# HTDerekLiu/surface_multigrid_code

Hardware: AMD Instinct MI355X
Metric: V-cycles/sec + fine-level SpMV GB/s (% HBM peak), 1M-vert mesh fp64 (higher is better)
Workload: dtype f64; 1 GPU; C3: bunny_15K_init x3 midpoint subdivision, 1011330 verts, 5 levels, M_bary+0.01(-L), fp64; n_verts=1011330, nnz=7079298, levels=5, smoother=gs, rhs_columns_per_gpu=1, parallelism=single GPU

## Files before the change

include/smg.h:

```cpp
#ifndef SMG_H
#define SMG_H

#ifdef __cplusplus
extern "C" {
#endif

#define SMG_VERSION 508

enum {
    SMG_OK = 0,
    SMG_ERR_INVALID = -1,
    SMG_ERR_NO_DEVICE = -2,
    SMG_ERR_HIP = -3,
    SMG_ERR_NONFINITE = -4,
    SMG_ERR_ALLOC = -5,
    SMG_ERR_IO = -6,
    SMG_ERR_REDUCE = -7
};

enum { SMG_HOST = 0, SMG_DEVICE = 1 };

enum { SMG_DEC_QSLIM = 0, SMG_DEC_MIDPOINT = 1, SMG_DEC_VERTEX_REMOVAL = 2 };

enum { SMG_SMOOTH_GS = 0, SMG_SMOOTH_JACOBI = 1, SMG_SMOOTH_HYBRID = 2, SMG_SMOOTH_CHEBYSHEV = 3, SMG_SMOOTH_HYBRID_CHEBYSHEV = 4 };

typedef struct smg_hierarchy smg_hierarchy;

typedef struct {
    double tol;
    int max_iter;
    int pre, post;
    int verbosity;
    int check_every;
    int use_graph;
    int precision;
    int smoother;
    double omega;
    int jacobi_max_rows;
    double cheby_fraction;
} smg_solve_opts;
void smg_solve_opts_default(smg_solve_opts *o);

int smg_version(void);
const char *smg_last_error(void);
int smg_device_count(void);
long long smg_device_bytes_live(void);
int smg_debug_device_bytes(const smg_hierarchy *h, char *buf, int cap);

smg_hierarchy *smg_hierarchy_create(int n_levels);
void smg_hierarchy_destroy(smg_hierarchy *h);
int smg_hierarchy_levels(const smg_hierarchy *h);
int smg_hierarchy_set_stream(smg_hierarchy *h, void *hip_stream);
int smg_hierarchy_set_smoother(smg_hierarchy *h, int smoother, double omega, int jacobi_max_rows);
int smg_hierarchy_set_chebyshev(smg_hierarchy *h, double cheby_fraction);
double smg_level_spectral_bound(const smg_hierarchy *h, int lv);
int smg_level_set_prolong(smg_hierarchy *h, int lv, int n_fine, int n_coarse, const int *rowptr, const int *col,
                          const double *val);
int smg_level_set_prolong_csc(smg_hierarchy *h, int lv, int n_fine, int n_coarse, const int *colptr,
                              const int *rowidx, const double *val);
int smg_level_set_mesh(smg_hierarchy *h, int lv, const double *V, int nV, const int *F, int nF);
int smg_level_get_mesh(const smg_hierarchy *h, int lv, int *nV, int *nF, double *V, int *F);

int smg_mg_precompute(const double *V, int nV, const int *F, int nF, float ratio, int nVCoarsest, int dec_type,
                      smg_hierarchy **out);
int smg_mg_precompute_capped(const double *V, int nV, const int *F, int nF, float ratio, int nVCoarsest, int dec_type,
                             float absorption_cap, smg_hierarchy **out);
int smg_mg_precompute_logged(const double *V, int nV, const int *F, int nF, float ratio, int nVCoarsest, int dec_type,
                             float absorption_cap, int keep_log, smg_hierarchy **out);
int smg_query_coarse_to_fine(const smg_hierarchy *h, int lv, int n, const int *face, const double *bary, int *out_face,
                             double *out_bary);
int smg_query_fine_to_coarse(const smg_hierarchy *h, int lv, int n, const int *face, const double *bary, int *out_face,
                             double *out_bary);
int smg_mg_precompute_subdiv(const double *V, int nV, const int *F, int nF, int n_sub, float ratio, int nVCoarsest,
                             int n_extra_levels, smg_hierarchy **out, double *V_out, int *F_out);

int smg_mg_precompute_block(const double *V, int nV, const int *F, int nF, float ratio, int nVCoarsest, int dec_type,
                            smg_hierarchy **out);
int smg_hierarchy_set_block_mode(smg_hierarchy *h, int mode);
int smg_hierarchy_block_size(const smg_hierarchy *h);
int smg_level_block_stats(const smg_hierarchy *h, int lv, long *n_blocks, long *n_block_slots, int *n_vertex_colors);
int smg_level_get_block_image(const smg_hierarchy *h, int lv, int *n_slices, int *n_panel_cols, int *slice_row, int *slice_off, int *slice_w,
                              int *col, double *val);
int smg_hierarchy_set_block_gs(smg_hierarchy *h, int min_rows);
int smg_level_get_block_gs_order(smg_hierarchy *h, int lv, int k, int *n_blocks, int *n_colors, int *color_ptr, int *blk_ptr, int *rows, double *stats);
int smg_hierarchy_set_wave_gs(smg_hierarchy *h, int mode);
int smg_hierarchy_set_memory_lean(smg_hierarchy *h, int on);
int smg_level_get_wave_gs_order(smg_hierarchy *h, int lv, int k, int *n_pieces, int *n_colors, int *color_ptr, int *piece_ptr, int *rows, double *stats);
int smg_hierarchy_create_union(const smg_hierarchy *const *members, int m, smg_hierarchy **out);
int smg_union_members(const smg_hierarchy *h);
int smg_union_member_rows(const smg_hierarchy *h, int member, int *first, int *count);
// ... 52 lines not shown
} smg_membrane_params;
void smg_membrane_params_default(smg_membrane_params *p);
typedef struct smg_membrane smg_membrane;
int smg_membrane_create(const smg_hierarchy *h, const double *V, int nV, const int *F, int nF, const smg_membrane_params *p, smg_membrane **out);
void smg_membrane_destroy(smg_membrane *m);
long long smg_membrane_device_bytes(const smg_membrane *m);
int smg_membrane_set_state(smg_membrane *m, const double *pos, const double *qdot, int memspace);
int smg_membrane_get_state(smg_membrane *m, double *pos, double *qdot, int memspace);
int smg_membrane_set_solver(smg_membrane *m, int pcg);
int smg_membrane_step(smg_membrane *m, const smg_solve_opts *opts, double *objective_his, double *alpha, int *cycles, int *n_newton);
int smg_membrane_lists(const int *F, int nF, int nV, int *n_blocks, int *n_contrib, int *bptr, int *bcol, int *c_ptr, int *c_src);
int smg_membrane_faces_host(const double *V0, const double *P, int nV, const int *F, int nF, const smg_membrane_params *p, int fix, double *W,
                            double *G, double *H);

int smg_solve_begin(smg_hierarchy *h, const double *RHS, int ld_rhs, const double *known_val, int ld_kv,
                    const double *z0, int ld_z0, int k, int memspace, const smg_solve_opts *opts);
int smg_solve_iter_residual(smg_hierarchy *h, double *d_sumsq);
int smg_solve_iter_cycle(smg_hierarchy *h, const double *d_sumsq);
int smg_solve_iter_cycle_speculative(smg_hierarchy *h);
int smg_solve_iter_commit(smg_hierarchy *h, const double *d_sumsq);
int smg_solve_poll(smg_hierarchy *h, int *done, int *n_his);
int smg_solve_end(smg_hierarchy *h, double *z, int ld_z, int memspace, double *r_his, int *n_his, int *converged);

typedef int (*smg_reduce_fn)(double *d_sumsq, int count, void *hip_stream, void *ctx);
int smg_solve_sharded(smg_hierarchy *h, const double *RHS, int ld_rhs, const double *known_val, int ld_kv, const double *z0,
                      int ld_z0, int k_local, int memspace, const smg_solve_opts *opts, smg_reduce_fn reduce, void *ctx,
                      double *z, int ld_z, double *r_his, int *n_his, int *converged);

int smg_level_rows(const smg_hierarchy *h, int lv);
int smg_vcycle(smg_hierarchy *h, const double *B, int pre, int post, int lv, double *u, int k);
int smg_apply_A(smg_hierarchy *h, int lv, const double *u, int k, double *Au);
int smg_restrict(smg_hierarchy *h, int lv, const double *x, int k, double *Rx);
int smg_prolong(smg_hierarchy *h, int lv, const double *x, int k, double *Px);
int smg_relax(smg_hierarchy *h, int lv, const double *B, int k, int iters, double *u);
int smg_coarse_solve(smg_hierarchy *h, const double *B, int k, double *u);
int smg_residual_norm(smg_hierarchy *h, int lv, const double *B, const double *u, int k, double *norm);

int smg_raw_spmv(smg_hierarchy *h, int lv, int mode, const double *x, const double *b, double *y, int k);
int smg_raw_relax(smg_hierarchy *h, int lv, const double *b, double *u, int k, int iters);
int smg_raw_spmv_f32(smg_hierarchy *h, int lv, const float *x, float *y, int k);
int smg_raw_outer_iteration(smg_hierarchy *h, int n_iter);
int smg_synchronize(smg_hierarchy *h);
int smg_bench_vcycle(smg_hierarchy *h, int lv, int k, int pre, int post, int reps, double *us_per_cycle);
int smg_bench_relax(smg_hierarchy *h, int lv, int k, int sweeps, int reps, double *us_per_call);

int smg_level_get_matrix(const smg_hierarchy *h, int lv, int which, int internal, int *n_rows, int *n_cols, int *nnz,
                         int *rowptr, int *col, double *val);
int smg_level_get_perm(const smg_hierarchy *h, int lv, int *perm);
int smg_level_get_colors(const smg_hierarchy *h, int lv, int *n_colors, int *color_ptr );
int smg_level_get_Adiag(const smg_hierarchy *h, int lv, double *diag);
int smg_get_unknown(const smg_hierarchy *h, int *n_unknown, int *unknown );
int smg_level_sell_stats(const smg_hierarchy *h, int lv, int which, long *stored, long *padded, int *n_slices);
int smg_level_first_colour_rows(const smg_hierarchy *h, int lv);
long smg_level_spmv_bytes(const smg_hierarchy *h, int lv, int k);
long smg_vcycle_bytes(const smg_hierarchy *h, int k, int pre, int post);

int smg_debug_check_tiling_plan(smg_hierarchy *h, int lv, int sweeps, int tile_rows, int *n_tiles, int *max_ext_rows, double *redundancy,
                                double *max_abs_diff);
int smg_debug_check_block_gs_plan(smg_hierarchy *h, int lv, int block_rows, int *n_blocks, int *n_colors, double *rim, double *fill, double *max_abs_diff);
int smg_debug_check_wave_gs_plan(smg_hierarchy *h, int lv, int piece_rows, int pieces_mode, int *n_pieces, int *n_colors, double *stats, double *max_abs_diff);
int smg_debug_raise_coarse_stall(smg_hierarchy *h);
int smg_debug_schur_solve_host(int n, const int *ptr, const int *col, const double *val, const double *b, double *x, int *n_blocks, int *n_sep);
int smg_debug_schur_partition(const smg_hierarchy *h, int *n_blocks, int *n_sep, int *block_of_row);
int smg_debug_check_sparse_cholesky(int n, const int *rowptr, const int *col, const double *val, long *factor_entries, int *dependency_depth,
                                    double *rel_residual);

int smg_debug_dense_geneig_host(int n, const double *A, const double *B, double *evals, double *V);

int smg_debug_eig_gram(int n, int m, int nb_a, const double *Sa, int nb_b, const double *Sb, const double *w, int sym, int done, double *G,
                       int *groups, int *guard_bad);
int smg_debug_eig_combine(int n, int m, int nb, const double *S, const double *AS, const double *C, int make_p, int done, double *X, double *AX,
                          double *P, double *AP, int *guard_bad);
int smg_debug_eig_residual(int n, int m, const double *X, const double *AX, const double *mass, const double *lam, int f32, int done, double *b0,
                           double *u0, float *b32, float *u32, double *res, int *groups, int *guard_bad);
enum { SMG_KRY_DOTS_ZR_ZQ = 0, SMG_KRY_DIRECTION = 1, SMG_KRY_DOTS_PQ = 2, SMG_KRY_STEP_DECIDE = 3, SMG_KRY_PRECOND_IN = 4, SMG_KRY_WIDEN = 5 };
int smg_debug_krylov(int op, int n, int k, double *v0, double *v1, double *v2, double *v3, float *e, double *s, int *restart, double tol, int done,
                     double *ctrl_d, int *ctrl_i, int *groups, int *guard_bad);
enum { SMG_F32_A = 0, SMG_F32_RESID = 1, SMG_F32_RESTRICT = 2, SMG_F32_PROLONG_ADD = 3, SMG_F32_RELAX = 4, SMG_F32_COARSE = 5, SMG_F32_VCYCLE = 6 };
int smg_debug_cycle_f32(smg_hierarchy *h, int op, int lv, int k, int pre, int post, int done, const float *in0, const float *in1, float *out,
                        int *inputs_changed);
enum { SMG_F32_RESIDUAL_TO_F32 = 0, SMG_F32_ADD_CORRECTION = 1 };
int smg_debug_convert_f32(smg_hierarchy *h, int op, int k, int done, const double *in64, const float *in32, double *out64, float *out_b32,
                          float *out_u32, int *inputs_changed);
enum { SMG_GEO_BASIS = 0, SMG_GEO_SCATTER = 1, SMG_GEO_DIVERGENCE = 2, SMG_GEO_SHIFT = 3 };
int smg_debug_geodesics(int op, int n, int nF, int k, const int *F, const int *m_ptr, const int *m_idx, const int *src_ptr, const int *src,
                        const double *in, double *W, double *Af, double *out, int ld_out, int *guard_bad);
enum { SMG_ARAP_COVARIANCE = 0, SMG_ARAP_ROTATIONS = 1, SMG_ARAP_RHS = 2, SMG_ARAP_VERTEX_ENERGY = 3, SMG_ARAP_ENERGY = 4 };
int smg_debug_arap(int op, int n, const int *rowptr, const int *col, const double *w, const double *P0, const double *P, const double *R_in,
                   double *out, int *guard_hits);

enum { SMG_MEM_REST = 0, SMG_MEM_FACES_RAW = 1, SMG_MEM_FACES = 2, SMG_MEM_ENERGY = 3, SMG_MEM_PRESSURE = 4, SMG_MEM_MATRIX = 5,
       SMG_MEM_GRADIENT = 6, SMG_MEM_OBJECTIVE = 7 };
int smg_debug_membrane(int op, int nV, int nF, const int *F, const double *V0, const double *P, const double *in, const smg_membrane_params *p,
                       double *out, int *guard_hits);

int smg_prof_enable(smg_hierarchy *h, int on);
int smg_prof_reset(smg_hierarchy *h);
int smg_prof_count(smg_hierarchy *h);
int smg_prof_get(smg_hierarchy *h, int idx, char *name, int name_cap, long *count, double *total_ms);

int smg_mesh_read(const char *path, double **V, int *nV, int **F, int *nF);
void smg_free(void *p);
int smg_mesh_normalize_unit_area(double *V, int nV, const int *F, int nF);
int smg_mesh_cotmatrix(const double *V, int nV, const int *F, int nF, int *nnz, int *rowptr, int *col, double *val);
int smg_mesh_massmatrix(const double *V, int nV, const int *F, int nF, int voronoi, double *diag);
int smg_mesh_boundary_loop(const int *F, int nF, int nV, int *loop, int *n_loop);
int smg_mesh_midpoint_upsample(int nV, const int *F, int nF, int *nE, int *S_rowptr, int *S_col, double *S_val,
                               int *NF);
int smg_mesh_torus(int nu, int nv, double R, double r, double *V, int *F);

#ifdef __cplusplus
}
#endif
#endif
```

surface_multigrid_code_amd/_lib.py:

```python
import ctypes as C
import os

HERE = os.path.dirname(os.path.abspath(__file__))
LIB_PATH = os.environ.get("SMG_LIB") or os.path.join(HERE, "lib", "libsmg.so")

SMG_HOST, SMG_DEVICE = 0, 1


class SolveOptsC(C.Structure):
    _fields_ = [("tol", C.c_double), ("max_iter", C.c_int), ("pre", C.c_int), ("post", C.c_int),
                ("verbosity", C.c_int), ("check_every", C.c_int), ("use_graph", C.c_int), ("precision", C.c_int),
                ("smoother", C.c_int), ("omega", C.c_double), ("jacobi_max_rows", C.c_int), ("cheby_fraction", C.c_double)]


class MembraneParamsC(C.Structure):
    _fields_ = [("young", C.c_double), ("poisson", C.c_double), ("thickness", C.c_double), ("mass_scale", C.c_double), ("dt", C.c_double),
                ("pressure", C.c_double), ("newton_iters", C.c_int), ("ls_c", C.c_double), ("ls_shrink", C.c_double),
                ("ls_min_alpha", C.c_double), ("eig_floor", C.c_double), ("eig_value", C.c_double)]


_lib = None


REDUCE_FN = C.CFUNCTYPE(C.c_int, C.c_void_p, C.c_int, C.c_void_p, C.c_void_p)


def load():
    global _lib
    if _lib is not None:
        return _lib
    if not os.path.exists(LIB_PATH):
        raise ImportError("libsmg.so not built: run `python -m surface_multigrid_code_amd.build` "
                          "(expected at %s); there is no CPU fallback" % LIB_PATH)
    L = C.CDLL(LIB_PATH, mode=C.RTLD_GLOBAL)
    ip, dp, vp, lp, fp = C.POINTER(C.c_int), C.POINTER(C.c_double), C.c_void_p, C.POINTER(C.c_long), C.POINTER(C.c_float)
    i, d, f = C.c_int, C.c_double, C.c_float
    sig = {
        "smg_version": (i, []),
        "smg_last_error": (C.c_char_p, []),
        "smg_device_count": (i, []),
        "smg_device_bytes_live": (C.c_longlong, []),
        "smg_solve_opts_default": (None, [C.POINTER(SolveOptsC)]),
        "smg_hierarchy_create": (vp, [i]),
        "smg_hierarchy_destroy": (None, [vp]),
        "smg_hierarchy_levels": (i, [vp]),
        "smg_hierarchy_set_stream": (i, [vp, vp]),
        "smg_hierarchy_set_smoother": (i, [vp, i, d, i]),
        "smg_hierarchy_set_chebyshev": (i, [vp, d]),
        "smg_level_spectral_bound": (d, [vp, i]),
        "smg_level_set_prolong": (i, [vp, i, i, i, ip, ip, dp]),
        "smg_level_set_prolong_csc": (i, [vp, i, i, i, ip, ip, dp]),
        "smg_level_set_mesh": (i, [vp, i, dp, i, ip, i]),
        "smg_level_get_mesh": (i, [vp, i, ip, ip, dp, ip]),
        "smg_mg_precompute": (i, [dp, i, ip, i, f, i, i, C.POINTER(vp)]),
        "smg_mg_precompute_capped": (i, [dp, i, ip, i, f, i, i, f, C.POINTER(vp)]),
        "smg_mg_precompute_logged": (i, [dp, i, ip, i, f, i, i, f, i, C.POINTER(vp)]),
        "smg_query_coarse_to_fine": (i, [vp, i, i, ip, dp, ip, dp]),
        "smg_query_fine_to_coarse": (i, [vp, i, i, ip, dp, ip, dp]),
        "smg_mg_precompute_block": (i, [dp, i, ip, i, f, i, i, C.POINTER(vp)]),
        "smg_hierarchy_save": (i, [vp, C.c_char_p]),
        "smg_hierarchy_load": (i, [C.c_char_p, C.POINTER(vp)]),
        "smg_mg_precompute_subdiv": (i, [dp, i, ip, i, i, f, i, i, C.POINTER(vp), dp, ip]),
        "smg_precompute": (i, [vp, i, ip, ip, dp, ip, i]),
        "smg_precompute_values_device": (i, [vp, vp]),
        "smg_assembler_create": (i, [ip, i, i, C.POINTER(vp)]),
        "smg_assembler_destroy": (None, [vp]),
        "smg_assembler_pattern": (i, [vp, ip, ip, ip]),
        "smg_assemble": (i, [vp, vp, i, d, d, vp, vp, vp, vp]),
        "smg_solve": (i, [vp, vp, i, vp, i, vp, i, i, i, C.POINTER(SolveOptsC), vp, i, dp, ip, ip]),
        "smg_solve_pcg": (i, [vp, vp, i, vp, i, vp, i, i, i, C.POINTER(SolveOptsC), vp, i, dp, ip, ip]),
        "smg_eigs": (i, [vp, vp, i, i, vp, i, i, C.POINTER(SolveOptsC), C.c_ulonglong, dp, vp, i, dp, ip, ip]),
        "smg_debug_dense_geneig_host": (i, [i, dp, dp, dp, dp]),
        "smg_debug_eig_gram": (i, [i, i, i, dp, i, dp, dp, i, i, dp, ip, ip]),
        "smg_debug_eig_combine": (i, [i, i, i, dp, dp, dp, i, i, dp, dp, dp, dp, ip]),
        "smg_debug_eig_residual": (i, [i, i, dp, dp, dp, dp, i, i, dp, dp, fp, fp, dp, ip, ip]),
        "smg_debug_krylov": (i, [i, i, i, dp, dp, dp, dp, fp, dp, ip, d, i, dp, ip, ip, ip]),
        "smg_debug_cycle_f32": (i, [vp, i, i, i, i, i, i, fp, fp, fp, ip]),
        "smg_debug_convert_f32": (i, [vp, i, i, i, dp, fp, dp, fp, fp, ip]),
        "smg_debug_geodesics": (i, [i, i, i, i, ip, ip, ip, ip, ip, dp, dp, dp, dp, i, ip]),
        "smg_geodesics_create": (i, [vp, dp, i, ip, i, d, i, C.POINTER(vp)]),
        "smg_geodesics_destroy": (None, [vp]),
        "smg_geodesics_time": (d, [vp]),
        "smg_geodesics_set_solver": (i, [vp, i, i]),
        "smg_geodesics_device_bytes": (C.c_longlong, [vp]),
        "smg_geodesics_solve": (i, [vp, i, ip, ip, i, C.POINTER(SolveOptsC), C.POINTER(SolveOptsC), vp, i, ip]),
        "smg_debug_arap": (i, [i, i, ip, ip, dp, dp, dp, dp, dp, ip]),
        "smg_arap_create": (i, [vp, dp, i, ip, i, ip, i, C.POINTER(vp)]),
        "smg_arap_destroy": (None, [vp]),
        "smg_arap_set_solver": (i, [vp, i]),
        "smg_arap_device_bytes": (C.c_longlong, [vp]),
        "smg_arap_solve": (i, [vp, vp, i, vp, i, i, i, d, C.POINTER(SolveOptsC), vp, i, dp, ip, ip]),
        "smg_debug_membrane": (i, [i, i, i, ip, dp, dp, dp, C.POINTER(MembraneParamsC), dp, ip]),
        "smg_membrane_params_default": (None, [C.POINTER(MembraneParamsC)]),
        "smg_membrane_create": (i, [vp, dp, i, ip, i, C.POINTER(MembraneParamsC), C.POINTER(vp)]),
        "smg_membrane_destroy": (None, [vp]),
        "smg_membrane_device_bytes": (C.c_longlong, [vp]),
        "smg_membrane_set_state": (i, [vp, vp, vp, i]),
        "smg_membrane_get_state": (i, [vp, vp, vp, i]),
        "smg_membrane_set_solver": (i, [vp, i]),
        "smg_membrane_step": (i, [vp, C.POINTER(SolveOptsC), dp, dp, ip, ip]),
        "smg_membrane_lists": (i, [ip, i, i, ip, ip, ip, ip, ip, ip]),
        "smg_membrane_faces_host": (i, [dp, dp, i, ip, i, C.POINTER(MembraneParamsC), i, dp, dp, dp]),
        "smg_solve_sharded": (i, [vp, vp, i, vp, i, vp, i, i, i, C.POINTER(SolveOptsC), REDUCE_FN, vp, vp, i, dp, ip, ip]),
        "smg_solve_begin": (i, [vp, vp, i, vp, i, vp, i, i, i, C.POINTER(SolveOptsC)]),
        "smg_solve_iter_residual": (i, [vp, vp]),
        "smg_solve_iter_cycle": (i, [vp, vp]),
        "smg_solve_iter_cycle_speculative": (i, [vp]),
        "smg_solve_iter_commit": (i, [vp, vp]),
        "smg_solve_poll": (i, [vp, ip, ip]),
        "smg_solve_end": (i, [vp, vp, i, i, dp, ip, ip]),
        "smg_level_rows": (i, [vp, i]),
        "smg_vcycle": (i, [vp, dp, i, i, i, dp, i]),
        "smg_apply_A": (i, [vp, i, dp, i, dp]),
        "smg_restrict": (i, [vp, i, dp, i, dp]),
        "smg_prolong": (i, [vp, i, dp, i, dp]),
        "smg_relax": (i, [vp, i, dp, i, i, dp]),
        "smg_coarse_solve": (i, [vp, dp, i, dp]),
        "smg_residual_norm": (i, [vp, i, dp, dp, i, dp]),
        "smg_raw_spmv": (i, [vp, i, i, vp, vp, vp, i]),
        "smg_raw_relax": (i, [vp, i, vp, vp, i, i]),
        "smg_raw_spmv_f32": (i, [vp, i, vp, vp, i]),
        "smg_raw_outer_iteration": (i, [vp, i]),
        "smg_synchronize": (i, [vp]),
        "smg_bench_vcycle": (i, [vp, i, i, i, i, i, dp]),
        "smg_bench_relax": (i, [vp, i, i, i, i, dp]),
        "smg_level_get_matrix": (i, [vp, i, i, i, ip, ip, ip, ip, ip, dp]),
        "smg_level_get_perm": (i, [vp, i, ip]),
        "smg_level_get_colors": (i, [vp, i, ip, ip]),
        "smg_level_get_Adiag": (i, [vp, i, dp]),
        "smg_get_unknown": (i, [vp, ip, ip]),
        "smg_level_sell_stats": (i, [vp, i, i, lp, lp, ip]),
        "smg_level_first_colour_rows": (i, [vp, i]),
        "smg_debug_check_tiling_plan": (i, [vp, i, i, i, ip, ip, dp, dp]),
        "smg_debug_check_sparse_cholesky": (i, [i, ip, ip, dp, lp, ip, dp]),
        "smg_hierarchy_set_coarse_dense_max": (i, [vp, i]),
        "smg_hierarchy_set_coarse_schur": (i, [vp, i, i]),
        "smg_debug_schur_solve_host": (i, [i, ip, ip, dp, dp, dp, ip, ip]),
        "smg_debug_schur_partition": (i, [vp, ip, ip, ip]),
        "smg_hierarchy_set_block_gs": (i, [vp, i]),
        "smg_hierarchy_set_wave_gs": (i, [vp, i]),
        "smg_hierarchy_set_memory_lean": (i, [vp, i]),
        "smg_hierarchy_create_union": (i, [C.POINTER(vp), i, C.POINTER(vp)]),
        "smg_union_members": (i, [vp]),
        "smg_union_member_rows": (i, [vp, i, ip, ip]),
        "smg_union_get_history": (i, [vp, i, dp, i, ip, ip]),
        "smg_debug_device_bytes": (i, [vp, C.c_char_p, i]),
        "smg_level_get_wave_gs_order": (i, [vp, i, i, ip, ip, ip, ip, ip, dp]),
        "smg_debug_check_wave_gs_plan": (i, [vp, i, i, i, ip, ip, dp, dp]),
        "smg_debug_raise_coarse_stall": (i, [vp]),
        "smg_debug_check_block_gs_plan": (i, [vp, i, i, ip, ip, dp, dp, dp]),
        "smg_level_get_block_gs_order": (i, [vp, i, i, ip, ip, ip, ip, ip, dp]),
        "smg_hierarchy_coarse_solver": (i, [vp, lp]),
        "smg_hierarchy_set_block_mode": (i, [vp, i]),
        "smg_hierarchy_block_size": (i, [vp]),
        "smg_level_block_stats": (i, [vp, i, lp, lp, ip]),
        "smg_level_get_block_image": (i, [vp, i, ip, ip, ip, ip, ip, ip, dp]),
        "smg_level_spmv_bytes": (C.c_long, [vp, i, i]),
        "smg_vcycle_bytes": (C.c_long, [vp, i, i, i]),
        "smg_prof_enable": (i, [vp, i]),
        "smg_prof_reset": (i, [vp]),
        "smg_prof_count": (i, [vp]),
# ... 22 lines not shown
```

surface_multigrid_code_amd/csrc/smg_cycle.cpp:

```cpp
#include <hip/hip_runtime.h>

#include <algorithm>
#include <chrono>
#include <cmath>
#include <cstdarg>
#include <cstdio>
#include <cstdlib>
#include <cstring>
#include <functional>
#include <memory>
#include <numeric>
#include <string>
#include <thread>
#include <vector>

#include "smg_internal.hpp"

using namespace smg;


int smg::ensure_work(smg_hierarchy* h, int k)
{
    const int L = h->n_levels;
    if (k > h->kcap) {
// ... 172 lines not shown
            const double rho_new = 1.0 / (2.0 * sigma - rho);
            out[s].c1 = rho_new * rho;
            out[s].c2 = 2.0 * rho_new / delta;
            rho = rho_new;
        }
    }
}

template <typename T> struct Prec;
static inline int coarse_cols(const smg_hierarchy* h, int k) { return (h->coarse_cols > 0 && h->coarse_cols < k) ? h->coarse_cols : k; }

template <> struct Prec<double> {
    static double* b(Level& L) { return L.b.p; }
    static double* u(Level& L) { return L.u.p; }
    static double* r(Level& L) { return L.r.p; }
    static double* t(Level& L) { return L.t.p; }
    static double* d(Level& L) { return L.d.p; }
    static void set_d(FirstColour& fc, Level& L) { fc.d = L.d.p; }
    static const SellDev& A(Level& L) { return L.dA.view; }
    static const SellDev& G(Level& L) { return L.gs_on_transpose ? L.dAT.view : L.dA.view; }
    static const SellDev& P(Level& L) { return L.dP.view; }
    static const SellDev& PT(Level& L) { return L.dPT.view; }
    static bool has_vals(const SellDev& V) { return V.val != nullptr; }
    static hipError_t sell(SellMode m, const SellDev& V, int s0, int s1, const double* x, const double* bb, double* y, int k, const Ctrl* ctrl,
                           hipStream_t st, double* zero_rows = nullptr, const FirstColour* first = nullptr, double omega = 1.0)
    { return launch_sell(m, V, s0, s1, x, bb, y, k, ctrl, nullptr, nullptr, st, zero_rows, first, omega); }
    static hipError_t coarse(smg_hierarchy* h, Level& L, int k, const Ctrl* ctrl)
    {
        if (h->union_m > 0) return launch_blockdiag_gemv_add(h->un.view, h->d_Ainv.p, h->nc, L.b.p, L.u.p, k, ctrl, h->stream);
        if (h->coarse_sparse) return launch_sparse_coarse_solve(h->c_view, L.b.p, L.u.p, k, ctrl, h->stream);
        if (h->coarse_schur) return launch_schur_solve(h->sch.view, L.b.p, L.u.p, k, ctrl, h->stream);
        return launch_dense_gemv_add(h->d_Ainv.p, h->nc, h->nc_pad, L.b.p, L.u.p, coarse_cols(h, k), k, ctrl, h->stream, h->d_sympart.p);
    }
    static hipError_t opA(smg_hierarchy* h, Level& L, bool smoother_image, SellMode m, int s0, int s1, const double* x, const double* bb, double* y, int k,
                          const Ctrl* ctrl, const FirstColour* fc = nullptr, double omega = 1.0)
    {
        if (h->bs == 3) {
            const Bsr3Dev& V = (smoother_image && L.gs_on_transpose) ? L.bAT.view : L.bA.view;
            return launch_bsr3(m, V, s0, s1 < 0 ? V.n_slices : s1, x, bb, y, k, ctrl, nullptr, nullptr, h->stream, omega, fc ? fc->c1 : 0.0, fc ? fc->d : nullptr);
        }
        const SellDev& V = smoother_image ? G(L) : A(L);
        return sell(m, V, s0, s1 < 0 ? V.n_slices : s1, x, bb, y, k, ctrl, h->stream, nullptr, fc, omega);
    }
};
template <> struct Prec<float> {
    static float* b(Level& L) { return L.b32.p; }
    static float* u(Level& L) { return L.u32.p; }
    static float* r(Level& L) { return L.r32.p; }
    static float* t(Level& L) { return L.t32.p; }
    static float* d(Level& L) { return L.d32.p; }
    static void set_d(FirstColour& fc, Level& L) { fc.df = L.d32.p; }
    static const SellDev& A(Level& L) { return L.dA32; }
    static const SellDev& G(Level& L) { return L.gs_on_transpose ? L.dAT32 : L.dA32; }
    static const SellDev& P(Level& L) { return L.dP32; }
    static const SellDev& PT(Level& L) { return L.dPT32; }
    static bool has_vals(const SellDev& V) { return V.valf != nullptr; }
    static hipError_t sell(SellMode m, const SellDev& V, int s0, int s1, const float* x, const float* bb, float* y, int k, const Ctrl* ctrl,
                           hipStream_t st, float* zero_rows = nullptr, const FirstColour* first = nullptr, double omega = 1.0)
    { return launch_sell_f32(m, V, s0, s1, x, bb, y, k, ctrl, st, zero_rows, first, omega); }
    static hipError_t coarse(smg_hierarchy* h, Level& L, int k, const Ctrl* ctrl)
    {
        if (h->coarse_schur) return launch_schur_solve_f32(h->sch.view, L.b32.p, L.u32.p, k, ctrl, h->stream);
        return launch_dense_gemv_add_f32(h->d_Ainv32.p, h->nc, h->nc_pad, L.b32.p, L.u32.p, coarse_cols(h, k), k, ctrl, h->stream, (float*)h->d_sympart.p);
    }
    static hipError_t opA(smg_hierarchy* h, Level& L, bool smoother_image, SellMode m, int s0, int s1, const float* x, const float* bb, float* y, int k,
                          const Ctrl* ctrl, const FirstColour* fc = nullptr, double omega = 1.0)
    {
        if (h->bs == 3) {
            const Bsr3Dev& V = (smoother_image && L.gs_on_transpose) ? L.bAT.view : L.bA.view;
            return launch_bsr3_f32(m, V, s0, s1 < 0 ? V.n_slices : s1, x, bb, y, k, ctrl, h->stream, omega, fc ? fc->c1 : 0.0, fc ? fc->df : nullptr);
        }
        const SellDev& V = smoother_image ? G(L) : A(L);
        return sell(m, V, s0, s1 < 0 ? V.n_slices : s1, x, bb, y, k, ctrl, h->stream, nullptr, fc, omega);
    }
};

static const std::vector<int>& colour_slices(const smg_hierarchy* h, const Level& Lv)
{
    if (h->bs == 3) return (Lv.gs_on_transpose ? Lv.bAT : Lv.bA).color_slice_ptr;
    return (Lv.gs_on_transpose ? Lv.dAT : Lv.dA).color_slice_ptr;
}

template <typename T>
static int enqueue_gs(smg_hierarchy* h, int lv, const SweepPlan& sp, const T* b, T* u, int k, int iters, const Ctrl* ctrl, int first = FIRST_NONE, T* t = nullptr)
{
    Level& Lv = h->lv[lv];
    ProfGuard pg(h, "MG: relaxation");
    if (const WgsBuf* W = sp.wave) {
        for (int it = 0; it < iters; it++)
            for (size_t c = 0; c + 1 < W->color_ptr.size(); c++)
                HIPCHK(launch_wgs(W->view, W->color_ptr[c], W->color_ptr[c + 1], (const double*)b, (double*)u, k, ctrl, h->stream));
        return SMG_OK;
    }
    if (const BgsBuf* Q = sp.block) {
        for (int it = 0; it < iters; it++)
            for (size_t c = 0; c + 1 < Q->color_ptr.size(); c++)
                HIPCHK(launch_bgs(Q->view, Q->color_ptr[c], Q->color_ptr[c + 1], (const double*)b, (double*)u, k, ctrl, h->stream));
        return SMG_OK;
    }
    const std::vector<int>& cs = colour_slices(h, Lv);
    for (int it = first == FIRST_SWEEP ? 1 : 0; it < iters; it++)
        for (size_t c = (it == 0 && first == FIRST_LAUNCH) ? 1 : 0; c + 1 < cs.size(); c++) {
            if (it == 1 && first == FIRST_SWEEP) HIPCHK(Prec<T>::sell(SELL_GS_OOP, Prec<T>::G(Lv), cs[c], cs[c + 1], t, b, u, k, ctrl, h->stream));
            else HIPCHK(Prec<T>::opA(h, Lv, true, SELL_GS, cs[c], cs[c + 1], u, b, u, k, ctrl));
        }
    return SMG_OK;
}

template <typename T>
static int enqueue_gs_tiled(smg_hierarchy* h, const TiledDev& plan, const T* b, T* const buf[2], int* cur, int k, const Ctrl* ctrl)
{
    ProfGuard pg(h, "MG: relaxation");
    HIPCHK(launch_tiled_gs(plan, (const double*)buf[*cur], (const double*)b, (double*)buf[1 - *cur], k, ctrl, h->stream));
    *cur ^= 1;
    return SMG_OK;
}

template <typename T>
static int enqueue_jacobi(smg_hierarchy* h, int lv, const T* b, T* const buf[2], int* cur, int k, int iters, const Ctrl* ctrl)
{
    Level& Lv = h->lv[lv];
    ProfGuard pg(h, "MG: relaxation");
    for (int it = 0; it < iters; it++) {
        HIPCHK(Prec<T>::opA(h, Lv, true, SELL_JACOBI, 0, -1, buf[*cur], b, buf[1 - *cur], k, ctrl, nullptr, h->omega));
        *cur ^= 1;
    }
    return SMG_OK;
}

template <typename T>
static int enqueue_cheby(smg_hierarchy* h, int lv, const T* b, T* const buf[2], int* cur, int k, int iters, const Ctrl* ctrl, bool first_done = false)
{
    if (iters <= 0) return SMG_OK;
    Level& Lv = h->lv[lv];
    ProfGuard pg(h, "MG: relaxation");
    std::vector<ChebyCoef> cf;
    cheby_coefs(Lv.lam, h->cheby_fraction, iters + 1, cf);
    for (int s = first_done ? 1 : 0; s <= iters; s++) {
        FirstColour fc;
        Prec<T>::set_d(fc, Lv);
        fc.c1 = cf[s].c1;
        HIPCHK(Prec<T>::opA(h, Lv, true, SELL_CHEBY, 0, -1, buf[*cur], b, buf[1 - *cur], k, ctrl, &fc, cf[s].c2));
        *cur ^= 1;
    }
    return SMG_OK;
}

static bool fuse_first_colour() { static const int on = env_int("SMG_FUSE_FIRST", 1); return on != 0; }

template <typename T>
static int enqueue_vcycle_t(smg_hierarchy* h, int lv, int k, int pre, int post, const Ctrl* ctrl, int first = FIRST_NONE)
{
    const bool first_done = first != FIRST_NONE;
    const int L = h->n_levels;
    Level& Lv = h->lv[lv];
    if (lv == L - 1) {
        ProfGuard pg(h, "MG: coarse solve");
        HIPCHK(Prec<T>::coarse(h, Lv, k, ctrl));
        return SMG_OK;
    }
    Level& Lc = h->lv[lv + 1];
    const int kind = level_kind(h, lv);
    const bool jac = kind != LV_GS;
    T* const buf[2] = {Prec<T>::u(Lv), Prec<T>::t(Lv)};
    int cur = 0;
    const bool fp64 = std::is_same<T, double>::value;
    const SweepPlan sp_pre = sweep_plan(h, lv, k, pre, fp64, first), sp_post = sweep_plan(h, lv, k, post, fp64, FIRST_NONE);
    int rc;
    if (kind == LV_JACOBI) {
        if (first_done) cur = 1;
        rc = enqueue_jacobi<T>(h, lv, Prec<T>::b(Lv), buf, &cur, k, pre - (first_done ? 1 : 0), ctrl);
    } else if (kind == LV_CHEBY) {
        if (first_done) cur = 1;
        rc = enqueue_cheby<T>(h, lv, Prec<T>::b(Lv), buf, &cur, k, pre, ctrl, first_done);
    } else if (sp_pre.tiled) rc = enqueue_gs_tiled<T>(h, *sp_pre.tiled, Prec<T>::b(Lv), buf, &cur, k, ctrl);
    else rc = enqueue_gs<T>(h, lv, sp_pre, Prec<T>::b(Lv), buf[0], k, pre, ctrl, first, buf[1]);
    if (rc) return rc;
    {
        ProfGuard pg(h, "MG: residual");
        HIPCHK(Prec<T>::opA(h, Lv, false, SELL_RESID, 0, -1, buf[cur], Prec<T>::b(Lv), Prec<T>::r(Lv), k, ctrl));
    }
    const SellBuf& Gc = Lc.gs_on_transpose ? Lc.dAT : Lc.dA;
    const int kind_c = level_kind(h, lv + 1);
    const bool jac_c = kind_c != LV_GS;
    const bool fuse = h->bs == 1 && sweep_plan(h, lv + 1, k, pre, fp64, FIRST_NONE).colours() && fuse_first_colour() && lv + 1 < L - 1 && pre > 0 && Prec<T>::has_vals(Prec<T>::G(Lc)) && (jac_c ? Gc.n_all > 0 : Gc.n_first > 0);
    const int kt = k * h->bs;
    {
        ProfGuard pg(h, "MG: restrict");
        FirstColour fc;
        if (fuse) {
            fc.diag_slot = Gc.diag_slot.p; fc.n_first = jac_c ? Gc.n_all : Gc.n_first;
            fc.val = Prec<T>::G(Lc).val; fc.valf = Prec<T>::G(Lc).valf;
            fc.jacobi = kind_c == LV_CHEBY ? 2 : (jac_c ? 1 : 0); fc.omega = h->omega;
            if (kind_c == LV_CHEBY) {
                std::vector<ChebyCoef> cf;
                cheby_coefs(Lc.lam, h->cheby_fraction, 1, cf);
                fc.omega = cf[0].c2;
                Prec<T>::set_d(fc, Lc);
            }
        }
        T* init = (fuse && jac_c) ? Prec<T>::t(Lc) : Prec<T>::u(Lc);
        HIPCHK(Prec<T>::sell(SELL_AX, Prec<T>::PT(Lc), 0, Prec<T>::PT(Lc).n_slices, Prec<T>::r(Lv), nullptr, Prec<T>::b(Lc), kt, ctrl, h->stream, init,
                             fuse ? &fc : nullptr));
    }
    rc = enqueue_vcycle_t<T>(h, lv + 1, k, pre, post, ctrl, fuse ? FIRST_LAUNCH : FIRST_NONE);
    if (rc) return rc;
    {
        ProfGuard pg(h, "MG: prolong");
        int dst = cur;
        const int flips = sp_post.tiled ? 1 : kind == LV_CHEBY ? (post > 0 ? post + 1 : 0) : post;
        if ((jac || sp_post.tiled) && ((cur + flips) & 1)) dst = 1 - cur;
        if (!jac && !sp_post.tiled && cur == 1) dst = 0;
        HIPCHK(Prec<T>::sell(SELL_ADD, Prec<T>::P(Lc), 0, Prec<T>::P(Lc).n_slices, Prec<T>::u(Lc), buf[cur], buf[dst], kt, ctrl, h->stream));
        cur = dst;
    }
    if (kind == LV_CHEBY) return enqueue_cheby<T>(h, lv, Prec<T>::b(Lv), buf, &cur, k, post, ctrl);
    if (jac) return enqueue_jacobi<T>(h, lv, Prec<T>::b(Lv), buf, &cur, k, post, ctrl);
    if (sp_post.tiled) return enqueue_gs_tiled<T>(h, *sp_post.tiled, Prec<T>::b(Lv), buf, &cur, k, ctrl);
    return enqueue_gs<T>(h, lv, sp_post, Prec<T>::b(Lv), buf[0], k, post, ctrl);
}

int smg::enqueue_vcycle(smg_hierarchy* h, int k, const Ctrl* ctrl, int first)
{
    if (h->precision == 1) return enqueue_vcycle_t<float>(h, 0, k, h->pre, h->post, ctrl);
    return enqueue_vcycle_t<double>(h, 0, k, h->pre, h->post, ctrl, first);
}

int smg::apply_A(smg_hierarchy* h, int lv, SellMode mode, const double* x, const double* b, double* y, int k, const Ctrl* ctrl)
{
    HIPCHK(Prec<double>::opA(h, h->lv[lv], false, mode, 0, -1, x, b, y, k, ctrl));
    return SMG_OK;
}


static int enqueue_relax(smg_hierarchy* h, int lv, const double* b, double* u, int k, int iters, const Ctrl* ctrl)
{
    Level& Lv = h->lv[lv];
    const int kind = level_kind(h, lv);
    const SweepPlan sp = sweep_plan(h, lv, k, iters, true, FIRST_NONE);
    if (kind == LV_GS && !sp.tiled) return enqueue_gs<double>(h, lv, sp, b, u, k, iters, ctrl);
    double* const buf[2] = {u, Lv.t.p};
    int cur = 0;
    int rc = kind == LV_GS ? enqueue_gs_tiled<double>(h, *sp.tiled, b, buf, &cur, k, ctrl)
             : kind == LV_CHEBY ? enqueue_cheby<double>(h, lv, b, buf, &cur, k, iters, ctrl) : enqueue_jacobi<double>(h, lv, b, buf, &cur, k, iters, ctrl);
    if (rc) return rc;
    if (cur == 1) HIPCHK(hipMemcpyAsync(u, Lv.t.p, (size_t)Lv.n * k * sizeof(double), hipMemcpyDeviceToDevice, h->stream));
    return SMG_OK;
}

bool smg::head_fusable(smg_hierarchy* h, int k)
{
    static const int on = env_int("SMG_FUSE_HEAD", 1);
    if (!on || h->precision != 0 || h->n_levels < 2 || h->prof_on || h->bs != 1 || h->union_m > 0) return false;
    Level& L0 = h->lv[0];
    if (L0.gs_on_transpose) return false;
    if (!sweep_plan(h, 0, k, h->pre, true, FIRST_NONE).colours()) return false;
    const int kind = level_kind(h, 0);
    return kind == LV_GS ? h->pre >= 2 : h->pre >= 1;
}

int smg::enqueue_residual_ss(smg_hierarchy* h, int k, bool fuse_decide, double* sumsq_out)
{
    Level& L0 = h->lv[0];
    int nb = 0;
    if (h->head_fuse) {
        ProfGuard pg(h, "MG: relaxation");
        const int kind = level_kind(h, 0);
        const SellDev& G = L0.dA.view;
        if (kind == LV_GS) {
            const std::vector<int>& cs = L0.dA.color_slice_ptr;
            for (size_t c = 0; c + 1 < cs.size(); c++) {
                int nbc = 0;
                HIPCHK(launch_sell(SELL_GS_HEAD, G, cs[c], cs[c + 1], L0.u.p, L0.b.p, L0.t.p, k, h->d_ctrl.p, h->d_partials.p + nb, &nbc, h->stream));
                nb += nbc;
            }
        } else if (kind == LV_JACOBI) {
            HIPCHK(launch_sell(SELL_JACOBI_HEAD, G, 0, G.n_slices, L0.u.p, L0.b.p, L0.t.p, k, h->d_ctrl.p, h->d_partials.p, &nb, h->stream, nullptr, nullptr, h->omega));
        } else {
            std::vector<ChebyCoef> cf;
            cheby_coefs(L0.lam, h->cheby_fraction, h->pre + 1, cf);
            FirstColour fc;
            fc.d = L0.d.p;
            fc.c1 = cf[0].c1;
            HIPCHK(launch_sell(SELL_CHEBY_HEAD, G, 0, G.n_slices, L0.u.p, L0.b.p, L0.t.p, k, h->d_ctrl.p, h->d_partials.p, &nb, h->stream, nullptr, &fc, cf[0].c2));
        }
        if (fuse_decide) HIPCHK(launch_ss_finalize_decide(h->d_partials.p, nb, h->d_ctrl.p, h->stream));
        else HIPCHK(launch_ss_finalize(h->d_partials.p, nb, h->d_ctrl.p, h->stream, sumsq_out));
        return SMG_OK;
    }
    ProfGuard pg(h, "MG: outer residual");
    if (h->union_m > 0) {
        if (!fuse_decide) return fail(SMG_ERR_INVALID, "a union handle runs through smg_solve / smg_solve_begin + smg_raw_outer_iteration (no split-phase iteration: its members stop one by one)");
        HIPCHK(launch_sell(SELL_RESID, L0.dA.view, 0, L0.dA.view.n_slices, L0.u.p, L0.b.p, L0.r.p, k, h->d_ctrl.p, nullptr, nullptr, h->stream));
        HIPCHK(launch_union_sumsq_decide(h->un.view, L0.r.p, L0.u.p, k, h->d_ctrl.p, h->stream));
        return SMG_OK;
    }
// ... 326 lines not shown
        const Ctrl* ctrl = h->d_ctrl.p;
        const int L = h->n_levels;
        Level& Lv = h->lv[lv];
        int changed = 0;
        std::vector<float> before, after;
        auto uploaded = [&]() -> int { return done ? snapshot_f32(h, before) : SMG_OK; };
        switch (op) {
            case SMG_F32_A:
                if ((rc = put_block<float>(h, lv, in0, k, Lv.u32.p))) return rc;
                if ((rc = put_block<float>(h, lv, out, k, Lv.r32.p)) || (rc = uploaded())) return rc;
                HIPCHK(Prec<float>::opA(h, Lv, false, SELL_AX, 0, -1, Lv.u32.p, nullptr, Lv.r32.p, k, ctrl));
                if ((rc = block_changed<float>(h, lv, Lv.u32.p, k, in0, &changed))) return rc;
                rc = get_block<float>(h, lv, Lv.r32.p, k, out);
                break;
            case SMG_F32_RESID:
                if ((rc = put_block<float>(h, lv, in0, k, Lv.b32.p))) return rc;
                if ((rc = put_block<float>(h, lv, in1, k, Lv.u32.p))) return rc;
                if ((rc = put_block<float>(h, lv, out, k, Lv.r32.p)) || (rc = uploaded())) return rc;
                HIPCHK(Prec<float>::opA(h, Lv, false, SELL_RESID, 0, -1, Lv.u32.p, Lv.b32.p, Lv.r32.p, k, ctrl));
                if ((rc = block_changed<float>(h, lv, Lv.b32.p, k, in0, &changed))) return rc;
                if ((rc = block_changed<float>(h, lv, Lv.u32.p, k, in1, &changed))) return rc;
                rc = get_block<float>(h, lv, Lv.r32.p, k, out);
                break;
            case SMG_F32_RESTRICT: {
                Level& Lc = h->lv[lv + 1];
                const size_t cc = (size_t)Lc.n * k;
                if ((rc = put_block<float>(h, lv, in0, k, Lv.r32.p))) return rc;
                if ((rc = put_block<float>(h, lv + 1, out, k, Lc.b32.p))) return rc;
                if ((rc = put_block<float>(h, lv + 1, out + cc, k, Lc.u32.p)) || (rc = uploaded())) return rc;
                HIPCHK(Prec<float>::sell(SELL_AX, Prec<float>::PT(Lc), 0, Prec<float>::PT(Lc).n_slices, Lv.r32.p, nullptr, Lc.b32.p, k * h->bs, ctrl, h->stream, Lc.u32.p,
                                         nullptr));
                if ((rc = block_changed<float>(h, lv, Lv.r32.p, k, in0, &changed))) return rc;
                if ((rc = get_block<float>(h, lv + 1, Lc.b32.p, k, out))) return rc;
                rc = get_block<float>(h, lv + 1, Lc.u32.p, k, out + cc);
                break;
            }
            case SMG_F32_PROLONG_ADD: {
                Level& Lc = h->lv[lv + 1];
                if ((rc = put_block<float>(h, lv + 1, in0, k, Lc.u32.p))) return rc;
                if ((rc = put_block<float>(h, lv, out, k, Lv.u32.p)) || (rc = uploaded())) return rc;
                HIPCHK(Prec<float>::sell(SELL_ADD, Prec<float>::P(Lc), 0, Prec<float>::P(Lc).n_slices, Lc.u32.p, Lv.u32.p, Lv.u32.p, k * h->bs, ctrl, h->stream));
                if ((rc = block_changed<float>(h, lv + 1, Lc.u32.p, k, in0, &changed))) return rc;
                rc = get_block<float>(h, lv, Lv.u32.p, k, out);
                break;
            }
            case SMG_F32_RELAX: {
                if ((rc = put_block<float>(h, lv, in0, k, Lv.b32.p))) return rc;
                if ((rc = put_block<float>(h, lv, out, k, Lv.u32.p))) return rc;
                if (level_is_jacobi(h, lv) && (rc = put_block<float>(h, lv, out, k, Lv.t32.p))) return rc;
                float* res = nullptr;
                if ((rc = uploaded())) return rc;
                if ((rc = enqueue_relax_f32(h, lv, k, pre, ctrl, &res))) return rc;
                if ((rc = block_changed<float>(h, lv, Lv.b32.p, k, in0, &changed))) return rc;
                rc = get_block<float>(h, lv, res, k, out);
                break;
            }
            case SMG_F32_COARSE:
                if ((rc = put_block<float>(h, lv, in0, k, Lv.b32.p))) return rc;
                if ((rc = put_block<float>(h, lv, out, k, Lv.u32.p)) || (rc = uploaded())) return rc;
                HIPCHK(Prec<float>::coarse(h, Lv, k, ctrl));
                if ((rc = block_changed<float>(h, lv, Lv.b32.p, k, in0, &changed))) return rc;
                rc = get_block<float>(h, lv, Lv.u32.p, k, out);
                break;
            case SMG_F32_VCYCLE:
                if ((rc = put_block<float>(h, lv, in0, k, Lv.b32.p))) return rc;
                if ((rc = put_block<float>(h, lv, out, k, Lv.u32.p))) return rc;
                if (lv < L - 1 && level_is_jacobi(h, lv) && (rc = put_block<float>(h, lv, out, k, Lv.t32.p))) return rc;
                if ((rc = uploaded())) return rc;
                if ((rc = enqueue_vcycle_t<float>(h, lv, k, pre, post, ctrl))) return rc;
                if ((rc = block_changed<float>(h, lv, Lv.b32.p, k, in0, &changed))) return rc;
                rc = get_block<float>(h, lv, Lv.u32.p, k, out);
                break;
        }
        if (rc) return rc;
        if (done) {
            if ((rc = snapshot_f32(h, after))) return rc;
            if (before.size() != after.size() || std::memcmp(before.data(), after.data(), after.size() * sizeof(float)) != 0) changed |= 4;
        }
        if (inputs_changed) *inputs_changed = changed;
        return SMG_OK;
    });
}

extern "C" int smg_debug_convert_f32(smg_hierarchy* h, int op, int k, int done, const double* in64, const float* in32, double* out64, float* out_b32,
                                     float* out_u32, int* inputs_changed)
{
    return guarded("smg_debug_convert_f32", [&]() -> int {
        if (!h) return fail(SMG_ERR_INVALID, "smg_debug_convert_f32: null handle");
        if (op != SMG_F32_RESIDUAL_TO_F32 && op != SMG_F32_ADD_CORRECTION) return fail(SMG_ERR_INVALID, "smg_debug_convert_f32: unknown op %d", op);
        if (op == SMG_F32_RESIDUAL_TO_F32 ? (!in64 || !out_b32 || !out_u32) : (!in32 || !out64)) return fail(SMG_ERR_INVALID, "smg_debug_convert_f32: missing array");
        int rc = piece_prolog(h, 0, k, "smg_debug_convert_f32", false);
        if (rc) return rc;
        DeviceScope dsc(h->device);
        if ((rc = ensure_fp32(h, k))) return rc;
        HookCtrlReset reset_on_exit{h};
        if ((rc = hook_ctrl(h, done))) return rc;
        const Ctrl* ctrl = h->d_ctrl.p;
        Level& L0 = h->lv[0];
        const size_t cnt = (size_t)L0.n * k;
        int changed = 0;
        auto tail_fill = [&](void* p, size_t have, size_t elem, int byte) -> int {
            if (have > cnt) HIPCHK(hipMemsetAsync((char*)p + cnt * elem, byte, (have - cnt) * elem, h->stream));
            return SMG_OK;
        };
        auto tail_check = [&](const void* p, size_t have, size_t elem) -> int {
            if (have <= cnt) return SMG_OK;
            std::vector<unsigned char> t((have - cnt) * elem);
            HIPCHK(hipMemcpyAsync(t.data(), (const char*)p + cnt * elem, t.size(), hipMemcpyDeviceToHost, h->stream));
            HIPCHK(hipStreamSynchronize(h->stream));
            for (unsigned char c : t) if (c != 0x5B) { changed |= 2; break; }
            return SMG_OK;
        };
        if (op == SMG_F32_RESIDUAL_TO_F32) {
            if (h->n_levels < 2) return fail(SMG_ERR_INVALID, "smg_debug_convert_f32: a one-level handle has no residual vector");
            if ((rc = put_block<double>(h, 0, in64, k, L0.r.p))) return rc;
            if ((rc = put_block<float>(h, 0, out_b32, k, L0.b32.p))) return rc;
            if ((rc = put_block<float>(h, 0, out_u32, k, L0.u32.p))) return rc;
            if ((rc = tail_fill(L0.b32.p, L0.b32.n, sizeof(float), 0x5B)) || (rc = tail_fill(L0.u32.p, L0.u32.n, sizeof(float), 0x5B))) return rc;
            HIPCHK(launch_residual_to_f32(L0.b32.p, L0.u32.p, L0.r.p, cnt, ctrl, h->stream));
            if ((rc = tail_check(L0.b32.p, L0.b32.n, sizeof(float))) || (rc = tail_check(L0.u32.p, L0.u32.n, sizeof(float)))) return rc;
            if ((rc = tail_fill(L0.b32.p, L0.b32.n, sizeof(float), 0)) || (rc = tail_fill(L0.u32.p, L0.u32.n, sizeof(float), 0))) return rc;
            if ((rc = block_changed<double>(h, 0, L0.r.p, k, in64, &changed))) return rc;
            if ((rc = get_block<float>(h, 0, L0.b32.p, k, out_b32))) return rc;
            if ((rc = get_block<float>(h, 0, L0.u32.p, k, out_u32))) return rc;
        } else {
            if ((rc = put_block<double>(h, 0, out64, k, L0.u.p))) return rc;
            if ((rc = put_block<float>(h, 0, in32, k, L0.u32.p))) return rc;
            if ((rc = tail_fill(L0.u.p, L0.u.n, sizeof(double), 0x5B))) return rc;
            HIPCHK(launch_add_correction(L0.u.p, L0.u32.p, cnt, ctrl, h->stream));
            if ((rc = tail_check(L0.u.p, L0.u.n, sizeof(double)))) return rc;
            if ((rc = tail_fill(L0.u.p, L0.u.n, sizeof(double), 0))) return rc;
            if ((rc = block_changed<float>(h, 0, L0.u32.p, k, in32, &changed))) return rc;
            if ((rc = get_block<double>(h, 0, L0.u.p, k, out64))) return rc;
        }
        if (inputs_changed) *inputs_changed = changed;
        return SMG_OK;
    });
}

extern "C" int smg_raw_spmv(smg_hierarchy* h, int lv, int mode, const double* x, const double* b, double* y, int k)
{
    int rc = check_ready(h, "smg_raw_spmv");
    if (rc) return rc;
    DeviceScope dsc(h->device);
    if (lv < 0 || lv >= h->n_levels - 1 || k < 1 || (mode != SELL_AX && mode != SELL_RESID && mode != SELL_ADD))
        return fail(SMG_ERR_INVALID, "smg_raw_spmv: bad level/mode");
    Level& Lv = h->lv[lv];
    if (h->bs == 3) {
        if (mode == SELL_ADD) return fail(SMG_ERR_INVALID, "smg_raw_spmv: y += A x is not available on block (3-DOF) hierarchies");
        HIPCHK(launch_bsr3((SellMode)mode, Lv.bA.view, 0, Lv.bA.view.n_slices, x, b, y, k, nullptr, nullptr, nullptr, h->stream));
        return SMG_OK;
    }
    HIPCHK(launch_sell((SellMode)mode, Lv.dA.view, 0, Lv.dA.view.n_slices, x, b, y, k, nullptr, nullptr, nullptr, h->stream));
    return SMG_OK;
}

extern "C" int smg_raw_spmv_f32(smg_hierarchy* h, int lv, const float* x, float* y, int k)
{
    int rc = check_ready(h, "smg_raw_spmv_f32");
    if (rc) return rc;
    DeviceScope dsc(h->device);
    if (lv < 0 || lv >= h->n_levels - 1 || k < 1) return fail(SMG_ERR_INVALID, "smg_raw_spmv_f32: bad level");
    if ((rc = ensure_work(h, k))) return rc;
    if ((rc = ensure_fp32(h, k))) return rc;
    Level& Lv = h->lv[lv];
    HIPCHK(launch_sell_f32(SELL_AX, Lv.dA32, 0, Lv.dA32.n_slices, x, nullptr, y, k, nullptr, h->stream));
// ... 43 lines not shown
```

surface_multigrid_code_amd/csrc/smg_device.hip:

```cpp
#include <hip/hip_runtime.h>

#include <cstdlib>
#include <type_traits>

#include "smg_device.hpp"
#include "smg_device_inl.hpp"
#include "smg_gj_inl.hpp"

namespace smg {


__device__ int g_never_done = 0;
const int* never_done()
{
    static const int* p = nullptr;
    if (!p) { void* q = nullptr; if (hipGetSymbolAddress(&q, HIP_SYMBOL(g_never_done)) == hipSuccess) p = (const int*)q; }
    return p;
}


template <typename T> struct CoarseInit { T* u; const T* gs_val; const int* diag_slot; int n_first; int jacobi; T omega; T* d; T c1; int codes; T tab[4]; };
template <typename T> __device__ __forceinline__ T code_val(const CoarseInit<T>& z, int cw)
{
    const T lo = (cw & 1) ? z.tab[1] : z.tab[0], hi = (cw & 1) ? z.tab[3] : z.tab[2];
    return (cw & 2) ? hi : lo;
}

template <int MODE, int KB, typename T, int W0C = -1, int WPB = 4, bool CODED = false>
__global__ __launch_bounds__(64 * WPB) void k_sell(const int* a_col, const T* a_val, const int* a_order, const int* a_slice_off, int a_stride,
                                              int a_w_lo, int s_begin, int s_end, int n_blocks, int use_order, const T* x,
                                              const int* a_slice_row, const int* a_slice_w, const T* b, T* y, int ld, const int* done,
                                              double* partials, CoarseInit<T> z)
{
    struct { const int *slice_row, *slice_off, *slice_w, *order, *col; int stride, w_lo; } A = {a_slice_row, a_slice_off, a_slice_w, a_order,
                                                                                               a_col, a_stride, a_w_lo};
    constexpr int C = 64;
    const int lane = threadIdx.x & 63;
    const int wave = threadIdx.x >> 6;
    constexpr int wpb = WPB;
    constexpr bool GS = sell_is_gs(MODE), OOP = sell_is_oop(MODE), JAC = sell_is_jacobi(MODE), CHEB = sell_is_cheby(MODE), HEAD = sell_is_head(MODE);
    int bid;
    if (GS && n_blocks < 0) { if (blockIdx.x & 7) return; bid = blockIdx.x >> 3; }
    else bid = xcd_remap(blockIdx.x, n_blocks);
    const int ls = __builtin_amdgcn_readfirstlane(s_begin + bid * wpb + wave);
    double ss = 0.0;
    int stop = 0;
    if (ls < s_end) {
        const int s = (!GS && use_order) ? A.order[ls] : ls;
        const int W0 = W0C >= 0 ? W0C : (A.w_lo < 8 ? A.w_lo : 8);
        const int off0 = (W0C >= 0 || A.stride) ? s * A.stride : A.slice_off[s];
        const int* cp = A.col + (size_t)off0 * C + lane;
        const T* vp = CODED ? nullptr : a_val + (size_t)off0 * C + lane;
        constexpr int U = W0C > 8 ? W0C : 8;
        int c0[U];
        T v0[U];
#pragma unroll
        for (int t = 0; t < U; t++) {
            if (t < W0) { c0[t] = cp[(size_t)t * C]; v0[t] = CODED ? (T)0 : vp[(size_t)t * C]; }
            else { c0[t] = -1; v0[t] = (T)0; }
        }
        {
            size_t keep = (size_t)x ^ (size_t)A.slice_row ^ (size_t)A.slice_w ^ (size_t)b ^ (size_t)y ^ (size_t)done ^ (size_t)ld;
            if (MODE == SELL_AX) keep ^= (size_t)z.u ^ (size_t)z.gs_val ^ (size_t)z.diag_slot ^ (size_t)z.n_first ^ (size_t)z.jacobi ^ (size_t)z.d;
            if (CHEB) keep ^= (size_t)z.d;
            asm("" : "+s"(keep));
            if (keep == 0x5a5a5a5a5a5a5a5bull) return;
        }
        stop = load_flag(done);
        const int row0 = A.slice_row[s];
        const int nrow = A.slice_row[s + 1] - row0;
        const int w = A.slice_w[s];
        const int rowb = row0 + lane;
        const int split = OOP ? A.slice_row[s_begin] : 0;
        T acc[KB];
        T accr[KB];
        T diag = (T)1;
        T xi[KB];
        T dold[KB];
        T bv[KB];
        const bool live = lane < nrow;
        T zd = (T)1;
        if (MODE == SELL_AX && live && rowb < z.n_first) zd = z.gs_val[z.diag_slot[rowb]];
#pragma unroll
        for (int q = 0; q < KB; q++) {
            acc[q] = (T)0; accr[q] = (T)0; xi[q] = (T)0; dold[q] = (T)0;
            if (MODE == SELL_AX) bv[q] = (T)0;
            else bv[q] = live ? b[(size_t)rowb * ld + q] : (T)0;
            if (CHEB && live && z.c1 != (T)0) dold[q] = z.d[(size_t)rowb * ld + q];
        }
        auto consume = [&](const int (&cw)[U], const T (&vw)[U]) {
            int c[U];
            T v[U];
#pragma unroll
            for (int t = 0; t < U; t++) {
                if constexpr (CODED) { c[t] = cw[t] >> 2; v[t] = code_val<T>(z, cw[t]); }
                else { c[t] = cw[t]; v[t] = vw[t]; }
            }
            T xv[U][KB];
            T xo[MODE == SELL_GS_HEAD ? U : 1][KB];
#pragma unroll
            for (int t = 0; t < U; t++) {
                const bool use = (c[t] >= 0) && !(GS && c[t] == rowb);
                if constexpr (MODE == SELL_GS_HEAD) {
                    gather_kb<KB, T>(x + (size_t)c[t] * ld, c[t] >= 0, xo[t]);
                    gather_kb<KB, T>((const T*)y + (size_t)c[t] * ld, use && c[t] < split, xv[t]);
                } else if constexpr (MODE == SELL_GS_OOP) {
                    gather_kb<KB, T>((c[t] < split ? (const T*)y : x) + (size_t)c[t] * ld, use, xv[t]);
                } else {
                    gather_kb<KB, T>(x + (size_t)c[t] * ld, use, xv[t]);
                }
            }
#pragma unroll
            for (int t = 0; t < U; t++) {
                if (c[t] >= 0) {
                    if (HEAD) {
#pragma unroll
                        for (int q = 0; q < KB; q++) accr[q] += v[t] * (MODE == SELL_GS_HEAD ? xo[t][q] : xv[t][q]);
                    }
                    if (GS && c[t] == rowb) {
                        diag = v[t];
                    } else if ((JAC || CHEB) && c[t] == rowb) {
                        diag = v[t];
#pragma unroll
                        for (int q = 0; q < KB; q++) xi[q] = xv[t][q];
                    } else {
#pragma unroll
                        for (int q = 0; q < KB; q++) acc[q] += v[t] * ((MODE == SELL_GS_HEAD && c[t] >= split) ? xo[t][q] : xv[t][q]);
                    }
                }
            }
        };
        if (W0 > 0) consume(c0, v0);
        for (int j0 = W0; j0 < w; j0 += U) {
            int c[U];
            T v[U];
#pragma unroll
            for (int t = 0; t < U; t++) {
                if ((j0 + t) < w) { c[t] = cp[(size_t)(j0 + t) * C]; v[t] = CODED ? (T)0 : vp[(size_t)(j0 + t) * C]; }
                else { c[t] = -1; v[t] = (T)0; }
            }
            consume(c, v);
        }
        if (live && !stop) {
            const size_t o = (size_t)rowb * ld;
#pragma unroll
            for (int q = 0; q < KB; q++) {
                if (MODE == SELL_AX) {
                    y[o + q] = acc[q];
                    if (z.u) {
                        const T t = acc[q] / zd;
                        if (z.jacobi == 2) { const T dn = z.omega * (t - (T)0); z.u[o + q] = (T)0 + dn; z.d[o + q] = dn; }
                        else z.u[o + q] = rowb < z.n_first ? (z.jacobi ? (T)0 + z.omega * (t - (T)0) : t) : (T)0;
                    }
                }
                else if (MODE == SELL_RESID) y[o + q] = bv[q] - acc[q];
                else if (MODE == SELL_ADD) y[o + q] = bv[q] + acc[q];
                else if (GS) y[o + q] = (bv[q] - acc[q]) / diag;
                else if (JAC) { const T t = (bv[q] - acc[q]) / diag; y[o + q] = xi[q] + z.omega * (t - xi[q]); }
                else if (CHEB) {
                    const T t = (bv[q] - acc[q]) / diag;
                    const T r = t - xi[q];
                    const T dn = z.c1 != (T)0 ? z.c1 * dold[q] + z.omega * r : z.omega * r;
                    y[o + q] = xi[q] + dn;
                    z.d[o + q] = dn;
                }
                else { const double t = (double)(bv[q] - acc[q]); ss += t * t; if (MODE == SELL_RESID_BOTH) y[o + q] = bv[q] - acc[q]; }
                if (HEAD) { const double t = (double)(bv[q] - accr[q]); ss += t * t; }
            }
        }
    }
    if (sell_has_ss(MODE)) {
        __shared__ double red[16];
#pragma unroll
        for (int o = 32; o > 0; o >>= 1) ss += __shfl_down(ss, o, 64);
        if (lane == 0) red[wave] = ss;
        __syncthreads();
        if (threadIdx.x == 0 && !stop) {
            double t = 0.0;
            for (int i2 = 0; i2 < wpb; i2++) t += red[i2];
            partials[HEAD ? bid : (int)blockIdx.x] = t;
        }
    }
}

template <int MODE, int KB, int NBMAX>
__global__ __launch_bounds__(256) void k_sell_deep(const int* a_col, const double* a_val, const int* a_order, const int* a_slice_off, int a_stride, int s_begin, int s_end,
                                                   int n_blocks, int use_order, const double* x, const int* a_slice_row, const int* a_slice_w, const double* b, double* y, int ld,
                                                   const int* done, CoarseInit<double> z)
{
    constexpr int C = 64, S = NBMAX * 8;
    const int lane = threadIdx.x & 63, wave = threadIdx.x >> 6;
    const int bid = xcd_remap(blockIdx.x, n_blocks);
    const int ls = __builtin_amdgcn_readfirstlane(s_begin + bid * 4 + wave);
    if (ls >= s_end) return;
    const int s = use_order ? a_order[ls] : ls;
    const int stop = load_flag(done);
    const int oz = __builtin_amdgcn_mbcnt_lo(~0u, 0u) >> 6;
    const int row0 = a_slice_row[s + oz], nrow = a_slice_row[s + 1 + oz] - row0, w = a_slice_w[s + oz];
    const int off0 = a_stride ? s * a_stride : a_slice_off[s + oz];
    const int rowb = row0 + lane;
    const bool live = lane < nrow;
    const int* cp = a_col + (size_t)off0 * C + lane;
    const double* vp = a_val + (size_t)off0 * C + lane;
    int c[S];
    double v[S];
#pragma unroll
    for (int bt = 0; bt < NBMAX; bt++) {
        if (bt * 8 < w) {
#pragma unroll
            for (int t = bt * 8; t < bt * 8 + 8; t++) {
                const int tt = t < w ? t : w - 1;
                c[t] = cp[(size_t)tt * C];
                v[t] = z.codes ? 0.0 : vp[(size_t)tt * C];
            }
        } else {
#pragma unroll
            for (int t = bt * 8; t < bt * 8 + 8; t++) { c[t] = -1; v[t] = 0.0; }
        }
    }
    double zd = 1.0, bv[KB];
    if (MODE == SELL_AX && live && rowb < z.n_first) zd = z.gs_val[z.diag_slot[rowb]];
#pragma unroll
    for (int q = 0; q < KB; q++) bv[q] = (MODE == SELL_RESID && live) ? b[(size_t)rowb * ld + q] : 0.0;
    if (z.codes) {
#pragma unroll
        for (int t = 0; t < S; t++) { v[t] = code_val<double>(z, c[t]); c[t] >>= 2; }
    }
    double xv[S][KB];
#pragma unroll
    for (int t = 0; t < S; t++) {
        const bool use = c[t] >= 0 && t < w;
        if (!use) v[t] = 0.0;
        gather_kb<KB, double>(x + (size_t)(use ? c[t] : 0) * ld, use, xv[t]);
    }
    double acc[KB];
#pragma unroll
    for (int q = 0; q < KB; q++) acc[q] = 0.0;
#pragma unroll
    for (int bt = 0; bt < NBMAX; bt++) {
// ... 284 lines not shown
static void launch_wide_one(const SellDev& A, int s_begin, int s_end, int use_order, const T* x, const T* b, T* y,
                            int k, const int* done, double* partials, CoarseInit<T> zero_rows, hipStream_t st, int* nb_out)
{
    const int ns = s_end - s_begin;
    if constexpr (KW < 64) if (wide_latency_variant(ns, KW)) {
        const int nb = (ns * KW + 3) / 4;
#define SMG_WIDE_LAT(UU) hipLaunchKernelGGL((k_sell_wide<MODE, KW, T, 1, UU>), dim3(nb), dim3(256), 0, st, A.col, host_vals<T>(A), A.order, A.slice_off, A.stride, \
                                             s_begin, s_end, nb, use_order, x, A.slice_row, A.slice_w, b, y, k, done, partials, zero_rows)
        if (A.w_max <= 8) SMG_WIDE_LAT(8);
        else if (A.w_max <= 16) SMG_WIDE_LAT(16);
        else SMG_WIDE_LAT(32);
#undef SMG_WIDE_LAT
        *nb_out = nb;
        return;
    }
    const int waves = ns * (KW / 2);
    const int nb = (waves + 3) / 4;
    hipLaunchKernelGGL((k_sell_wide<MODE, KW, T>), dim3(nb), dim3(256), 0, st, A.col, host_vals<T>(A), A.order, A.slice_off, A.stride, s_begin, s_end, nb, use_order, x,
                       A.slice_row, A.slice_w, b, y, k, done, partials, zero_rows);
    *nb_out = nb;
}

int sell_wide_blocks(int n_slices, int k)
{
    int tot = 0, c0 = 0;
    while (k - c0 >= 8) { int kw = 64; while (kw > k - c0) kw >>= 1; tot += (n_slices * kw + 3) / 4; c0 += kw; }
    return tot;
}

static constexpr int sell_wpb() { return 4; }
static int gs_wpb() { static const int v = getenv("SMG_GS_WPB") ? atoi(getenv("SMG_GS_WPB")) : 4; return v; }
int sell_blocks(int n_slices) { return (n_slices + sell_wpb() - 1) / sell_wpb(); }

template <int MODE, typename T, bool CODED>
static void launch_narrow(const SellDev& A, int kb, int nb, int ns, int grid, int nbarg, bool one_xcd, int s_begin, int s_end, int use_order, const T* xx,
                          const T* bb, T* yy, int k, const int* done, double* pp, const CoarseInit<T>& zz, hipStream_t st)
{
    switch (kb) {
        case 1: {
            const int w0 = A.stride > 0 ? (A.w_lo < 8 ? A.w_lo : 8) : -1;
            static const int pitch_env = getenv("SMG_PITCH_SPEC_MAX") ? atoi(getenv("SMG_PITCH_SPEC_MAX")) : -1;
            const int pitch_max = pitch_env >= 0 ? pitch_env : (sell_is_gs(MODE) ? 32 : 64);
            if (nb <= pitch_max && A.stride == 12 && w0 >= 7) hipLaunchKernelGGL((k_sell<MODE, 1, T, 12, 4, CODED>), dim3(grid), dim3(64 * sell_wpb()), 0, st, A.col, CODED ? nullptr : host_vals<T>(A), A.order, A.slice_off, A.stride, A.w_lo, s_begin, s_end, nbarg, use_order, xx, A.slice_row, A.slice_w, bb, yy, k, done, pp, zz);
            else if (!CODED && w0 == 7 && MODE == SELL_GS && !one_xcd && gs_wpb() == 8) hipLaunchKernelGGL((k_sell<MODE == SELL_GS ? MODE : SELL_GS, 1, T, 7, 8>), dim3((ns + 7) / 8), dim3(512), 0, st, A.col, CODED ? nullptr : host_vals<T>(A), A.order, A.slice_off, A.stride, A.w_lo, s_begin, s_end, (ns + 7) / 8, use_order, xx, A.slice_row, A.slice_w, bb, yy, k, done, pp, zz);
            else if (!CODED && w0 == 7 && MODE == SELL_GS && !one_xcd && gs_wpb() == 2) hipLaunchKernelGGL((k_sell<MODE == SELL_GS ? MODE : SELL_GS, 1, T, 7, 2>), dim3((ns + 1) / 2), dim3(128), 0, st, A.col, CODED ? nullptr : host_vals<T>(A), A.order, A.slice_off, A.stride, A.w_lo, s_begin, s_end, (ns + 1) / 2, use_order, xx, A.slice_row, A.slice_w, bb, yy, k, done, pp, zz);
            else if (w0 == 7) hipLaunchKernelGGL((k_sell<MODE, 1, T, 7, 4, CODED>), dim3(grid), dim3(64 * sell_wpb()), 0, st, A.col, CODED ? nullptr : host_vals<T>(A), A.order, A.slice_off, A.stride, A.w_lo, s_begin, s_end, nbarg, use_order, xx, A.slice_row, A.slice_w, bb, yy, k, done, pp, zz);
            else if (w0 == 8) hipLaunchKernelGGL((k_sell<MODE, 1, T, 8, 4, CODED>), dim3(grid), dim3(64 * sell_wpb()), 0, st, A.col, CODED ? nullptr : host_vals<T>(A), A.order, A.slice_off, A.stride, A.w_lo, s_begin, s_end, nbarg, use_order, xx, A.slice_row, A.slice_w, bb, yy, k, done, pp, zz);
            else if (w0 == 2) hipLaunchKernelGGL((k_sell<MODE, 1, T, 2, 4, CODED>), dim3(grid), dim3(64 * sell_wpb()), 0, st, A.col, CODED ? nullptr : host_vals<T>(A), A.order, A.slice_off, A.stride, A.w_lo, s_begin, s_end, nbarg, use_order, xx, A.slice_row, A.slice_w, bb, yy, k, done, pp, zz);
            else hipLaunchKernelGGL((k_sell<MODE, 1, T, -1, 4, CODED>), dim3(grid), dim3(64 * sell_wpb()), 0, st, A.col, CODED ? nullptr : host_vals<T>(A), A.order, A.slice_off, A.stride, A.w_lo, s_begin, s_end, nbarg, use_order, xx, A.slice_row, A.slice_w, bb, yy, k, done, pp, zz);
            break;
        }
        case 2:
            if (A.stride > 0 && A.w_lo == 7) hipLaunchKernelGGL((k_sell<MODE, 2, T, 7, 4, CODED>), dim3(grid), dim3(64 * sell_wpb()), 0, st, A.col, CODED ? nullptr : host_vals<T>(A), A.order, A.slice_off, A.stride, A.w_lo, s_begin, s_end, nbarg, use_order, xx, A.slice_row, A.slice_w, bb, yy, k, done, pp, zz);
            else hipLaunchKernelGGL((k_sell<MODE, 2, T, -1, 4, CODED>), dim3(grid), dim3(64 * sell_wpb()), 0, st, A.col, CODED ? nullptr : host_vals<T>(A), A.order, A.slice_off, A.stride, A.w_lo, s_begin, s_end, nbarg, use_order, xx, A.slice_row, A.slice_w, bb, yy, k, done, pp, zz);
            break;
        case 3:
            if (A.stride > 0 && A.w_lo == 7) hipLaunchKernelGGL((k_sell<MODE, 3, T, 7, 4, CODED>), dim3(grid), dim3(64 * sell_wpb()), 0, st, A.col, CODED ? nullptr : host_vals<T>(A), A.order, A.slice_off, A.stride, A.w_lo, s_begin, s_end, nbarg, use_order, xx, A.slice_row, A.slice_w, bb, yy, k, done, pp, zz);
            else hipLaunchKernelGGL((k_sell<MODE, 3, T, -1, 4, CODED>), dim3(grid), dim3(64 * sell_wpb()), 0, st, A.col, CODED ? nullptr : host_vals<T>(A), A.order, A.slice_off, A.stride, A.w_lo, s_begin, s_end, nbarg, use_order, xx, A.slice_row, A.slice_w, bb, yy, k, done, pp, zz);
            break;
        default:
            if (A.stride > 0 && A.w_lo == 7) hipLaunchKernelGGL((k_sell<MODE, 4, T, 7, 4, CODED>), dim3(grid), dim3(64 * sell_wpb()), 0, st, A.col, CODED ? nullptr : host_vals<T>(A), A.order, A.slice_off, A.stride, A.w_lo, s_begin, s_end, nbarg, use_order, xx, A.slice_row, A.slice_w, bb, yy, k, done, pp, zz);
            else hipLaunchKernelGGL((k_sell<MODE, 4, T, -1, 4, CODED>), dim3(grid), dim3(64 * sell_wpb()), 0, st, A.col, CODED ? nullptr : host_vals<T>(A), A.order, A.slice_off, A.stride, A.w_lo, s_begin, s_end, nbarg, use_order, xx, A.slice_row, A.slice_w, bb, yy, k, done, pp, zz);
            break;
    }
}

template <int MODE, typename T>
static hipError_t launch_sell_mode(const SellDev& A, int s_begin, int s_end_in, const T* x, const T* b, T* y,
                                   int k, const Ctrl* ctrl, double* partials, int* n_blocks, hipStream_t st, T* zero_rows, const FirstColour* first,
                                   double omega)
{
    int s_end = s_end_in;
    if (MODE == SELL_ADD && !b) b = y;
    const int ns = s_end - s_begin;
    const int nb = sell_blocks(ns);
    const int* done = ctrl ? &ctrl->done : never_done();
    static const int dbg_empty = getenv("SMG_DEBUG_EMPTY") ? atoi(getenv("SMG_DEBUG_EMPTY")) : 0;
    if (dbg_empty == 1) s_end = s_begin;
    const int use_order = (A.order && s_begin == 0 && s_end == A.n_slices) ? 1 : 0;
    if (n_blocks) *n_blocks = 0;
    if (ns <= 0) return hipSuccess;
    int c0 = 0;
    size_t poff = 0;
    {
        while (k - c0 >= 8) {
            int kw = 64;
            while (kw > k - c0) kw >>= 1;
            const T* xx = x ? x + c0 : nullptr;
            const T* bb = b ? b + c0 : nullptr;
            T* yy = y ? y + c0 : nullptr;
            double* pp = partials ? partials + poff : nullptr;
            const CoarseInit<T> zz = coarse_codes<T>(A, zero_rows, c0, first, omega);
            int wnb = 0;
            switch (kw) {
                case 64: launch_wide_one<MODE, 64, T>(A, s_begin, s_end, use_order, xx, bb, yy, k, done, pp, zz, st, &wnb); break;
                case 32: launch_wide_one<MODE, 32, T>(A, s_begin, s_end, use_order, xx, bb, yy, k, done, pp, zz, st, &wnb); break;
                case 16: launch_wide_one<MODE, 16, T>(A, s_begin, s_end, use_order, xx, bb, yy, k, done, pp, zz, st, &wnb); break;
                default: launch_wide_one<MODE, 8, T>(A, s_begin, s_end, use_order, xx, bb, yy, k, done, pp, zz, st, &wnb); break;
            }
            poff += (size_t)wnb;
            c0 += kw;
        }
    }
    static const int one_xcd_max = getenv("SMG_ONE_XCD_MAX") ? atoi(getenv("SMG_ONE_XCD_MAX")) : 32;
    const bool one_xcd = sell_is_gs(MODE) && nb <= one_xcd_max;
    const int grid = one_xcd ? nb * 8 : nb, nbarg = one_xcd ? -nb : nb;
    for (; c0 < k; c0 += 4) {
        const int kb = (k - c0) < 4 ? (k - c0) : 4;
        const T* xx = x ? x + c0 : nullptr;
        const T* bb = b ? b + c0 : nullptr;
        T* yy = y ? y + c0 : nullptr;
        double* pp = partials ? partials + poff : nullptr;
        const CoarseInit<T> zz = coarse_codes<T>(A, zero_rows, c0, first, omega);
        poff += (size_t)nb;
        if constexpr (std::is_same<T, double>::value && (MODE == SELL_AX || MODE == SELL_RESID)) {
            int kd = kb;
            if (kd == 4 && !deep_wanted(MODE, A.w_max, 4) && deep_wanted(MODE, A.w_max, 2)) kd = 2;
            if (deep_wanted(MODE, A.w_max, kd) || (kd > 1 && deep_wanted(MODE, A.w_max, 1))) {
                for (int cc = 0; cc < kb;) {
                    int kk = kb - cc;
                    while (kk > 1 && !deep_wanted(MODE, A.w_max, kk)) kk--;
                    const int nbm = A.w_max <= 24 ? 3 : A.w_max <= 40 ? 5 : 8;
                    const CoarseInit<T> zc = coarse_codes<T>(A, zero_rows, c0 + cc, first, omega);
#define SMG_DEEP_LAUNCH(KB, NB) hipLaunchKernelGGL((k_sell_deep<MODE, KB, NB>), dim3(nb), dim3(256), 0, st, A.col, A.val, A.order, A.slice_off, A.stride, s_begin, s_end, nb, use_order, \
                                                   xx ? xx + cc : nullptr, A.slice_row, A.slice_w, bb ? bb + cc : nullptr, yy + cc, k, done, zc)
                    if (nbm == 3) { if (kk == 1) SMG_DEEP_LAUNCH(1, 3); else if (kk == 2) SMG_DEEP_LAUNCH(2, 3); else SMG_DEEP_LAUNCH(3, 3); }
                    else if (nbm == 5) { if (kk == 1) SMG_DEEP_LAUNCH(1, 5); else SMG_DEEP_LAUNCH(2, 5); }
                    else SMG_DEEP_LAUNCH(1, 8);
#undef SMG_DEEP_LAUNCH
                    cc += kk;
                }
                continue;
            }
        }
        if constexpr (MODE == SELL_AX || MODE == SELL_ADD) {
            if (A.codes) { launch_narrow<MODE, T, true>(A, kb, nb, ns, grid, nbarg, one_xcd, s_begin, s_end, use_order, xx, bb, yy, k, done, pp, zz, st); continue; }
        }
        launch_narrow<MODE, T, false>(A, kb, nb, ns, grid, nbarg, one_xcd, s_begin, s_end, use_order, xx, bb, yy, k, done, pp, zz, st);
    }
    if (MODE == SELL_AX && A.long_n > 0 && s_begin == 0 && s_end_in == A.n_slices && host_long_vals<T>(A)) {
        const CoarseInit<T> zz = coarse_codes<T>(A, zero_rows, 0, first, omega);
        if (k >= 8) {
            const long waves = (long)A.long_n * ((k + 63) / 64);
            hipLaunchKernelGGL((k_long_ax_cols<T>), dim3((unsigned)((waves + 3) / 4)), dim3(256), 0, st, A.long_row, A.long_ptr, A.long_col, host_long_vals<T>(A), A.long_n, x, y,
                               k, k, done, zz);
        } else {
            const long waves = (long)A.long_n * k;
            hipLaunchKernelGGL((k_long_ax<T>), dim3((unsigned)((waves + 3) / 4)), dim3(256), 0, st, A.long_row, A.long_ptr, A.long_col, host_long_vals<T>(A), A.long_n, x, y, k, k,
                               done, zz);
        }
    }
    if (n_blocks) *n_blocks = (int)poff;
    return hipGetLastError();
}

template <typename T>
static hipError_t launch_sell_any(SellMode mode, const SellDev& A, int s_begin, int s_end, const T* x, const T* b,
                                  T* y, int k, const Ctrl* ctrl, double* partials, int* n_blocks, hipStream_t st,
                                  T* zero_rows, const FirstColour* first, double omega)
{
    switch (mode) {
        case SELL_JACOBI: return launch_sell_mode<SELL_JACOBI, T>(A, s_begin, s_end, x, b, y, k, ctrl, partials, n_blocks, st, zero_rows, first, omega);
        case SELL_CHEBY: return launch_sell_mode<SELL_CHEBY, T>(A, s_begin, s_end, x, b, y, k, ctrl, partials, n_blocks, st, zero_rows, first, omega);
        case SELL_AX: return launch_sell_mode<SELL_AX, T>(A, s_begin, s_end, x, b, y, k, ctrl, partials, n_blocks, st, zero_rows, first, omega);
        case SELL_RESID: return launch_sell_mode<SELL_RESID, T>(A, s_begin, s_end, x, b, y, k, ctrl, partials, n_blocks, st, zero_rows, first, omega);
        case SELL_RESID_SS:
            if constexpr (std::is_same<T, double>::value) return launch_sell_mode<SELL_RESID_SS, T>(A, s_begin, s_end, x, b, y, k, ctrl, partials, n_blocks, st, zero_rows, first, omega);
            else return hipErrorInvalidValue;
        case SELL_ADD: return launch_sell_mode<SELL_ADD, T>(A, s_begin, s_end, x, b, y, k, ctrl, partials, n_blocks, st, zero_rows, first, omega);
        case SELL_GS: return launch_sell_mode<SELL_GS, T>(A, s_begin, s_end, x, b, y, k, ctrl, partials, n_blocks, st, zero_rows, first, omega);
        case SELL_RESID_BOTH:
            if constexpr (std::is_same<T, double>::value) return launch_sell_mode<SELL_RESID_BOTH, T>(A, s_begin, s_end, x, b, y, k, ctrl, partials, n_blocks, st, zero_rows, first, omega);
            else return hipErrorInvalidValue;
        case SELL_GS_OOP:
            if constexpr (std::is_same<T, double>::value) return launch_sell_mode<SELL_GS_OOP, T>(A, s_begin, s_end, x, b, y, k, ctrl, partials, n_blocks, st, zero_rows, first, omega);
            else return hipErrorInvalidValue;
        case SELL_GS_HEAD:
            if constexpr (std::is_same<T, double>::value) return launch_sell_mode<SELL_GS_HEAD, T>(A, s_begin, s_end, x, b, y, k, ctrl, partials, n_blocks, st, zero_rows, first, omega);
            else return hipErrorInvalidValue;
        case SELL_JACOBI_HEAD:
            if constexpr (std::is_same<T, double>::value) return launch_sell_mode<SELL_JACOBI_HEAD, T>(A, s_begin, s_end, x, b, y, k, ctrl, partials, n_blocks, st, zero_rows, first, omega);
            else return hipErrorInvalidValue;
        case SELL_CHEBY_HEAD:
            if constexpr (std::is_same<T, double>::value) return launch_sell_mode<SELL_CHEBY_HEAD, T>(A, s_begin, s_end, x, b, y, k, ctrl, partials, n_blocks, st, zero_rows, first, omega);
            else return hipErrorInvalidValue;
    }
    return hipErrorInvalidValue;
}

hipError_t launch_sell(SellMode mode, const SellDev& A, int s_begin, int s_end, const double* x, const double* b,
                       double* y, int k, const Ctrl* ctrl, double* partials, int* n_blocks, hipStream_t st,
                       double* zero_rows, const FirstColour* first, double omega)
{
    return launch_sell_any<double>(mode, A, s_begin, s_end, x, b, y, k, ctrl, partials, n_blocks, st, zero_rows, first, omega);
}

hipError_t launch_sell_f32(SellMode mode, const SellDev& A, int s_begin, int s_end, const float* x, const float* b,
                           float* y, int k, const Ctrl* ctrl, hipStream_t st, float* zero_rows, const FirstColour* first, double omega)
{
    if ((!A.valf && !A.codes) || mode == SELL_RESID_SS || mode == SELL_RESID_BOTH || mode >= SELL_GS_OOP) return hipErrorInvalidValue;
    return launch_sell_any<float>(mode, A, s_begin, s_end, x, b, y, k, ctrl, nullptr, nullptr, st, zero_rows, first, omega);
}

__global__ __launch_bounds__(256) void k_gershgorin(const int* a_col, const double* a_val, const int* a_slice_row, const int* a_slice_off, const int* a_slice_w,
                                                    int stride, int n_slices, unsigned long long* out)
{
    const int lane = threadIdx.x & 63, s = blockIdx.x * 4 + (threadIdx.x >> 6);
    double ratio = 0.0;
    if (s < n_slices) {
        const int row0 = a_slice_row[s], nrow = a_slice_row[s + 1] - row0, w = a_slice_w[s];
        const size_t off = (size_t)(stride ? s * stride : a_slice_off[s]) * 64 + lane;
        double sum = 0.0, diag = 0.0;
        for (int j = 0; j < w; j++) {
            const int c = a_col[off + (size_t)j * 64];
            const double v = a_val[off + (size_t)j * 64];
            if (c >= 0) { sum += fabs(v); if (c == row0 + lane) diag = v; }
        }
        if (lane < nrow && diag > 0.0) ratio = sum / diag;
    }
#pragma unroll
    for (int o = 32; o > 0; o >>= 1) ratio = fmax(ratio, __shfl_down(ratio, o, 64));
    if (lane == 0 && ratio > 0.0) atomicMax(out, (unsigned long long)__double_as_longlong(ratio));
}
hipError_t launch_gershgorin(const SellDev& A, double* out, hipStream_t st)
{
    hipError_t e = hipMemsetAsync(out, 0, sizeof(double), st);
    if (e != hipSuccess || A.n_slices <= 0) return e;
    hipLaunchKernelGGL(k_gershgorin, dim3((A.n_slices + 3) / 4), dim3(256), 0, st, A.col, A.val, A.slice_row, A.slice_off, A.slice_w, A.stride, A.n_slices,
                       (unsigned long long*)out);
    return hipGetLastError();
}


__global__ __launch_bounds__(256) void k_ss_finalize(const double* partials, int n, Ctrl* ctrl, double* out)
{
    if (ctrl->done) return;
    __shared__ double red[256];
    double s = 0.0;
    for (int i = threadIdx.x; i < n; i += 256) s += partials[i];
    red[threadIdx.x] = s;
    __syncthreads();
    for (int o = 128; o > 0; o >>= 1) {
        if ((int)threadIdx.x < o) red[threadIdx.x] += red[threadIdx.x + o];
        __syncthreads();
    }
    if (threadIdx.x == 0) *out = red[0];
}

__global__ __launch_bounds__(256) void k_ss_finalize_decide(const double* partials, int n, Ctrl* ctrl)
{
    __shared__ double red[256];
    const int done = ctrl->done, n_his = ctrl->n_his, his_cap = ctrl->his_cap;
    const double tol = ctrl->tol;
    double* const r_his = ctrl->r_his;
    double s = 0.0;
#pragma unroll 8
    for (int i = threadIdx.x; i < n; i += 256) s += partials[i];
    if (done) return;
// ... 945 lines not shown
    const int row0 = slice_row[s], nrow = slice_row[s + 1] - row0;
    if (lane >= nrow) return;
    const int old = perm[row0 + lane];
    const int p0 = ptr[old], p1 = ptr[old + 1];
    const size_t base = (size_t)(stride ? s * stride : slice_off[s]) * 64 + lane;
    for (int p = p0; p < p1; p++) {
        const int j = col[p];
        const int c = iperm[j];
        int rank = 0;
        for (int q = p0; q < p1; q++) rank += iperm[col[q]] < c ? 1 : 0;
        int from = p;
        if (transposed) {
            int lo = ptr[j], hi = ptr[j + 1];
            while (lo < hi) { const int mid = (lo + hi) >> 1; if (col[mid] < old) lo = mid + 1; else hi = mid; }
            from = lo;
        }
        if (MAP) s_map[base + (size_t)rank * 64] = from;
        else {
            s_col[base + (size_t)rank * 64] = c;
            s_val[base + (size_t)rank * 64] = val[from];
        }
    }
}
hipError_t launch_sell_fill(const int* ptr, const int* col, const double* val, const int* perm, const int* iperm, const SellDev& S, size_t padded, hipStream_t st,
                            bool transposed)
{
    hipError_t e = hipMemsetAsync(const_cast<int*>(S.col), 0xFF, padded * sizeof(int), st);
    if (e == hipSuccess) e = hipMemsetAsync(const_cast<double*>(S.val), 0, padded * sizeof(double), st);
    if (e != hipSuccess || S.n_slices <= 0) return e;
    hipLaunchKernelGGL(k_sell_fill<false>, dim3((S.n_slices + 3) / 4), dim3(256), 0, st, ptr, col, val, perm, iperm, S.slice_row, S.slice_off, S.stride, S.n_slices,
                       transposed ? 1 : 0, const_cast<int*>(S.col), const_cast<double*>(S.val), (int*)nullptr);
    return hipGetLastError();
}
hipError_t launch_sell_fill_map(const int* ptr, const int* col, const int* perm, const int* iperm, const SellDev& S, size_t padded, bool transposed, int* map, hipStream_t st)
{
    hipError_t e = hipMemsetAsync(map, 0xFF, padded * sizeof(int), st);
    if (e != hipSuccess || S.n_slices <= 0) return e;
    hipLaunchKernelGGL(k_sell_fill<true>, dim3((S.n_slices + 3) / 4), dim3(256), 0, st, ptr, col, (const double*)nullptr, perm, iperm, S.slice_row, S.slice_off, S.stride,
                       S.n_slices, transposed ? 1 : 0, (int*)nullptr, (double*)nullptr, map);
    return hipGetLastError();
}

__global__ __launch_bounds__(256) void k_sell_encode(const int* __restrict__ s_col, const double* __restrict__ s_val, size_t n, double t0, double t1, double t2,
                                                     double t3, int n_tab, int* __restrict__ out, int* bad)
{
    const size_t i = (size_t)blockIdx.x * 256 + threadIdx.x;
    if (i >= n) return;
    const int c = s_col[i];
    if (c < 0) { out[i] = -1; return; }
    const long long b = __double_as_longlong(s_val[i]);
    const int code = b == __double_as_longlong(t0) ? 0 : (n_tab > 1 && b == __double_as_longlong(t1)) ? 1 : (n_tab > 2 && b == __double_as_longlong(t2)) ? 2
                   : (n_tab > 3 && b == __double_as_longlong(t3)) ? 3 : -1;
    if (code < 0 || c >= (1 << 29)) { atomicOr(bad, 1); out[i] = -1; return; }
    out[i] = (c << 2) | code;
}
hipError_t launch_sell_encode(const SellDev& S, size_t padded, const double* tab, int n_tab, int* out_col, int* bad, hipStream_t st)
{
    if (padded == 0) return hipSuccess;
    hipLaunchKernelGGL(k_sell_encode, dim3(grid1d(padded, 256)), dim3(256), 0, st, S.col, S.val, padded, tab[0], tab[1], tab[2], tab[3], n_tab, out_col, bad);
    return hipGetLastError();
}

__global__ __launch_bounds__(256) void k_sell_diag_slots(const int* __restrict__ slice_row, const int* __restrict__ slice_off, const int* __restrict__ slice_w, int stride,
                                                         int n_slices, const int* __restrict__ s_col, int* __restrict__ slot, int* first_missing)
{
    const int lane = threadIdx.x & 63, s = (int)blockIdx.x * 4 + (int)(threadIdx.x >> 6);
    if (s >= n_slices) return;
    const int row0 = slice_row[s], nrow = slice_row[s + 1] - row0;
    if (lane >= nrow) return;
    const int r = row0 + lane, w = slice_w[s];
    const size_t base = (size_t)(stride ? s * stride : slice_off[s]) * 64 + lane;
    int at = -1;
    for (int j = 0; j < w; j++) if (s_col[base + (size_t)j * 64] == r) { at = (int)(base + (size_t)j * 64); break; }
    slot[r] = at;
    if (at < 0) atomicMin(first_missing, r);
}
hipError_t launch_sell_diag_slots(const SellDev& S, int* slot, int* first_missing, hipStream_t st)
{
    if (S.n_slices <= 0) return hipSuccess;
    hipLaunchKernelGGL(k_sell_diag_slots, dim3((S.n_slices + 3) / 4), dim3(256), 0, st, S.slice_row, S.slice_off, S.slice_w, S.stride, S.n_slices, S.col, slot, first_missing);
    return hipGetLastError();
}

__global__ void k_nothing() {}
hipError_t warm_device_code(hipStream_t st)
{
    hipLaunchKernelGGL(k_nothing, dim3(1), dim3(64), 0, st);
    return hipGetLastError();
}

__global__ __launch_bounds__(256) void k_bit_symmetric(int n, const int* __restrict__ ptr, const int* __restrict__ col, const double* __restrict__ val, int* differs)
{
    const int i = blockIdx.x * blockDim.x + threadIdx.x;
    if (i >= n) return;
    int d = 0;
    for (int p = ptr[i]; p < ptr[i + 1]; p++) {
        const int j = col[p];
        if (j < 0 || j >= n) { d |= 2; continue; }
        int lo = ptr[j], hi = ptr[j + 1];
        while (lo < hi) { const int mid = (lo + hi) >> 1; if (col[mid] < i) lo = mid + 1; else hi = mid; }
        if (lo >= ptr[j + 1] || col[lo] != i) d |= 2;
        else if (__double_as_longlong(val[lo]) != __double_as_longlong(val[p])) d |= 1;
    }
    if (d) atomicOr(differs, d);
}
hipError_t launch_bit_symmetric(int n, const int* ptr, const int* col, const double* val, int* differs, hipStream_t st)
{
    hipError_t e = hipMemsetAsync(differs, 0, sizeof(int), st);
    if (e != hipSuccess || n <= 0) return e;
    hipLaunchKernelGGL(k_bit_symmetric, dim3(grid1d((size_t)n, 256)), dim3(256), 0, st, n, ptr, col, val, differs);
    return hipGetLastError();
}

hipError_t launch_gather_vals(double* dst, const double* src, const int* map, size_t n, hipStream_t st)
{
    if (n == 0) return hipSuccess;
    hipLaunchKernelGGL(k_gather_vals, dim3(grid1d(n, 256)), dim3(256), 0, st, dst, src, map, n);
    return hipGetLastError();
}
hipError_t launch_dense_from_csr(double* dense, int np, int n, const double* src, const long long* pos, int nnz, hipStream_t st)
{
    hipLaunchKernelGGL(k_dense_identity, dim3(grid1d((size_t)np * np, 256)), dim3(256), 0, st, dense, np, n);
    if (nnz > 0) hipLaunchKernelGGL(k_scatter_dense, dim3(grid1d(nnz, 256)), dim3(256), 0, st, dense, src, pos, nnz);
    return hipGetLastError();
}
hipError_t launch_scatter_dense(double* dense, const double* src, const long long* pos, int nnz, hipStream_t st)
{
    if (nnz > 0) hipLaunchKernelGGL(k_scatter_dense, dim3(grid1d(nnz, 256)), dim3(256), 0, st, dense, src, pos, nnz);
    return hipGetLastError();
}
hipError_t launch_dense_identity(double* dense, int np, int n, hipStream_t st)
{
    hipLaunchKernelGGL(k_dense_identity, dim3(grid1d((size_t)np * np, 256)), dim3(256), 0, st, dense, np, n);
    return hipGetLastError();
}
hipError_t launch_add_at(double* v, const int* where, int n, double c, hipStream_t st)
{
    if (n <= 0) return hipSuccess;
    hipLaunchKernelGGL(k_add_at, dim3(grid1d(n, 256)), dim3(256), 0, st, v, where, n, c);
    return hipGetLastError();
}

hipError_t launch_gather_in(double* dst, const double* src, const int* map, int n, int k, int kin, int ld_src, hipStream_t st)
{
    if ((size_t)n * k == 0) return hipSuccess;
    hipLaunchKernelGGL(k_gather_in, dim3(grid1d((size_t)n * kin, 256)), dim3(256), 0, st, dst, src, map, n, k, kin, ld_src);
    return hipGetLastError();
}
hipError_t launch_scatter_out(double* dst, const double* src, const int* map, int n, int k, int kin, int ld_dst, hipStream_t st)
{
    if ((size_t)n * k == 0) return hipSuccess;
    hipLaunchKernelGGL(k_scatter_out, dim3(grid1d((size_t)n * k, 256)), dim3(256), 0, st, dst, src, map, n, k, kin, ld_dst);
    return hipGetLastError();
}
hipError_t launch_scatter_cm(double* dst, const double* src, const int* idx, int n, int k, int ld_src, int ld_dst,
                             hipStream_t st)
{
    if ((size_t)n * k == 0) return hipSuccess;
    hipLaunchKernelGGL(k_scatter_cm, dim3(grid1d((size_t)n * k, 256)), dim3(256), 0, st, dst, src, idx, n, k, ld_src, ld_dst);
    return hipGetLastError();
}
hipError_t launch_gather_cm(double* dst, const double* src, const int* idx, int n, int k, int ld_src, int ld_dst,
                            hipStream_t st)
{
    if ((size_t)n * k == 0) return hipSuccess;
    hipLaunchKernelGGL(k_gather_cm, dim3(grid1d((size_t)n * k, 256)), dim3(256), 0, st, dst, src, idx, n, k, ld_src, ld_dst);
// ... 12 lines not shown
```

surface_multigrid_code_amd/csrc/smg_device.hpp:

```cpp
#pragma once
#include <hip/hip_runtime_api.h>

#include <cstdint>

namespace smg {

struct Ctrl {
    int done;
    int n_his;
    int status;
    int just_done;
    double sumsq;
    double tol;
    double* r_his;
    int his_cap;
    int pad_;
    double r_last, r_prev;
};

struct SellDev {
    int n_rows = 0, n_cols = 0, n_slices = 0;
    int C = 64;
    const int* slice_row = nullptr;
    const int* slice_off = nullptr;
    const int* slice_w = nullptr;
    int stride = 0;
    int w_lo = 0;
    int w_max = 0;
    const int* order = nullptr;
    const int* col = nullptr;
    const double* val = nullptr;
    const float* valf = nullptr;
    int codes = 0;
    double tab[4] = {0.0, 0.0, 0.0, 0.0};
    float tabf[4] = {0.0f, 0.0f, 0.0f, 0.0f};
    int long_n = 0;
    const int* long_row = nullptr;
    const int* long_ptr = nullptr;
    const int* long_col = nullptr;
    const double* long_val = nullptr;
    const float* long_valf = nullptr;
};

enum SellMode {
    SELL_AX = 0,
    SELL_RESID = 1,
    SELL_RESID_SS = 2,
    SELL_ADD = 3,
    SELL_GS = 4,
    SELL_RESID_BOTH = 5,
    SELL_JACOBI = 6,
    SELL_CHEBY = 7,
    SELL_GS_OOP = 8,
    SELL_GS_HEAD = 9,
    SELL_JACOBI_HEAD = 10,
    SELL_CHEBY_HEAD = 11,
};
constexpr bool sell_is_gs(int m) { return m == SELL_GS || m == SELL_GS_OOP || m == SELL_GS_HEAD; }
constexpr bool sell_is_oop(int m) { return m == SELL_GS_OOP || m == SELL_GS_HEAD; }
constexpr bool sell_is_jacobi(int m) { return m == SELL_JACOBI || m == SELL_JACOBI_HEAD; }
constexpr bool sell_is_cheby(int m) { return m == SELL_CHEBY || m == SELL_CHEBY_HEAD; }
constexpr bool sell_is_head(int m) { return m == SELL_GS_HEAD || m == SELL_JACOBI_HEAD || m == SELL_CHEBY_HEAD; }
constexpr bool sell_has_ss(int m) { return sell_is_head(m) || m == SELL_RESID_SS || m == SELL_RESID_BOTH; }

struct FirstColour {
    const int* diag_slot = nullptr;
    int n_first = 0;
    const double* val = nullptr;
    const float* valf = nullptr;
    int jacobi = 0;
    double omega = 1.0;
    double* d = nullptr;
    float* df = nullptr;
    double c1 = 0.0;
};
hipError_t launch_sell(SellMode mode, const SellDev& A, int s_begin, int s_end, const double* x, const double* b,
                       double* y, int k, const Ctrl* ctrl, double* partials, int* n_blocks, hipStream_t st,
                       double* zero_rows = nullptr, const FirstColour* first = nullptr, double omega = 1.0);
hipError_t launch_sell_f32(SellMode mode, const SellDev& A, int s_begin, int s_end, const float* x, const float* b,
                           float* y, int k, const Ctrl* ctrl, hipStream_t st, float* zero_rows = nullptr,
                           const FirstColour* first = nullptr, double omega = 1.0);
hipError_t launch_gershgorin(const SellDev& A, double* out, hipStream_t st);
struct Bsr3Dev {
    int n_vert = 0, n_slices = 0, w_max = 0;
    const int* slice_row = nullptr;
    const int* slice_off = nullptr;
    const int* slice_w = nullptr;
    const int* order = nullptr;
    const int* col = nullptr;
    const double* val = nullptr;
    const float* valf = nullptr;
};
hipError_t launch_bsr3(SellMode mode, const Bsr3Dev& A, int s_begin, int s_end, const double* x, const double* b, double* y, int k, const Ctrl* ctrl,
                       double* partials, int* n_blocks, hipStream_t st, double omega = 1.0, double c1 = 0.0, double* dvec = nullptr);
hipError_t launch_bsr3_f32(SellMode mode, const Bsr3Dev& A, int s_begin, int s_end, const float* x, const float* b, float* y, int k, const Ctrl* ctrl, hipStream_t st,
                           double omega = 1.0, double c1 = 0.0, float* dvec = nullptr);
hipError_t launch_bsr3_gershgorin(const Bsr3Dev& A, double* out, hipStream_t st);
int bsr3_blocks(int n_slices);
hipError_t launch_bsr3_fill(const int* ptr, const int* col, const double* val, const int* gptr, const int* gcol, const int* perm, const int* iperm, const Bsr3Dev& B,
                            size_t panel_cols, bool transposed, hipStream_t st);

struct BgsDev {
    int n_blocks = 0, n_colors = 0, xrows = 0;
    const int* hdr = nullptr;
    const int* xrow = nullptr;
    const int* ugrow = nullptr;
    const int* ulrow = nullptr;
    const double* udiag = nullptr;
    const int* eidx = nullptr;
    const double* eval = nullptr;
};
hipError_t launch_bgs(const BgsDev& P, int b_begin, int b_end, const double* b, double* u, int k, const Ctrl* ctrl, hipStream_t st);

struct WgsDev {
    int n_pieces = 0, n_colors = 0, rim_pitch = 0, nb_max = 0;
    const int* hdr = nullptr;
    const int* grow = nullptr;
    const int* meta = nullptr;
    const double* diag = nullptr;
    const int* rim = nullptr;
    const unsigned* eoff = nullptr;
    const double* eval = nullptr;
};
hipError_t launch_wgs(const WgsDev& P, int q_begin, int q_end, const double* b, double* u, int k, const Ctrl* ctrl, hipStream_t st);

struct UnionDev {
    int m = 0, his_cap = 0, max_rows = 0;
    const int* rows = nullptr;
    const int* rptr = nullptr;
    const int* crow_member = nullptr;
    const long long* moff = nullptr;
    const int* mlda = nullptr;
    const int* mrow0 = nullptr;
    double* ss = nullptr;
    double* his = nullptr;
    int* nhis = nullptr;
    int* done = nullptr;
    double* zsave = nullptr;
};
hipError_t launch_blockdiag_gemv_add(const UnionDev& U, const double* Ainv, int n, const double* b, double* u, int k, const Ctrl* ctrl, hipStream_t st);
hipError_t launch_union_sumsq_decide(const UnionDev& U, const double* r, const double* u, int k, Ctrl* ctrl, hipStream_t st);
hipError_t launch_union_restore(const UnionDev& U, double* u, int k, const Ctrl* ctrl, hipStream_t st);
// ... 24 lines not shown
hipError_t launch_sparse_coarse_solve(const SparseCholDev& F, const double* b, double* u, int k, const Ctrl* ctrl, hipStream_t st);
int sparse_coarse_work_cols(int k);

constexpr int SCHUR_M_MAX_DEV = 128;
struct SchurDev {
    int n = 0, nb = 0, ns = 0, ns_pad = 0;
    const int *irow = nullptr, *bsize = nullptr, *srow = nullptr, *sptr = nullptr, *sidx = nullptr, *aptr = nullptr, *ablk = nullptr, *apan = nullptr;
    double* arena = nullptr;
    float* arena32 = nullptr;
    long long off_D = 0, off_P = 0, off_W = 0, off_S = 0, off_C = 0;
    const long long *coff = nullptr, *pos = nullptr, *pos2 = nullptr, *ones = nullptr, *rdst = nullptr, *rdst2 = nullptr, *rsrc = nullptr;
    const int* rptr = nullptr;
    int nnz = 0, n_ones = 0, n_red = 0;
    double *g = nullptr, *xs = nullptr;
    float *g32 = nullptr, *xs32 = nullptr;
    double* sym_work = nullptr;
    double* gj_work = nullptr;
};
hipError_t launch_schur_factor(const SchurDev& F, const double* vals, hipStream_t st);
hipError_t launch_schur_check(const SchurDev& F, int* d_flag, hipStream_t st);
hipError_t launch_schur_solve(const SchurDev& F, const double* b, double* u, int k, const Ctrl* ctrl, hipStream_t st);
hipError_t launch_schur_solve_f32(const SchurDev& F, const float* b, float* u, int k, const Ctrl* ctrl, hipStream_t st);

int sell_blocks(int n_slices);
int sell_wide_blocks(int n_slices, int k);

int ss_partials_room();
hipError_t launch_ss_finalize(const double* partials, int n, Ctrl* ctrl, hipStream_t st, double* out = nullptr);
hipError_t launch_decide(Ctrl* ctrl, const double* sumsq, hipStream_t st);
hipError_t launch_decide_spec(Ctrl* ctrl, const double* sumsq, hipStream_t st);
hipError_t launch_copy_unless_done(double* dst, const double* src, size_t n, const Ctrl* ctrl, hipStream_t st);
hipError_t launch_restore_if_just_done(double* dst, const double* src, size_t n, const Ctrl* ctrl, hipStream_t st);
hipError_t launch_ss_finalize_decide(const double* partials, int n, Ctrl* ctrl, hipStream_t st);

enum { KS_RZ = 0, KS_RZ_PREV = 1, KS_ALPHA = 2, KS_BETA = 3, KS_SLOTS = 4 };
constexpr int KRY_MAX_GROUPS = 512;
struct KryDev {
    int n = 0, k = 0;
    int groups = 0;
    double* part = nullptr;
    double* s = nullptr;
    int* restart = nullptr;
};
int kry_groups(int n, int k);
hipError_t launch_kry_dots_zr_zq(const KryDev& K, const double* z, const double* r, const double* q, const Ctrl* ctrl, hipStream_t st);
hipError_t launch_kry_direction(const KryDev& K, const double* z, double* p, const Ctrl* ctrl, hipStream_t st);
hipError_t launch_kry_dots_pq(const KryDev& K, const double* p, const double* q, const Ctrl* ctrl, hipStream_t st);
hipError_t launch_kry_step_decide(const KryDev& K, double* x, double* r, const double* p, const double* q, Ctrl* ctrl, hipStream_t st);
hipError_t launch_kry_precond_in(const double* r, double* b0, double* u0, size_t cnt, const Ctrl* ctrl, hipStream_t st);
hipError_t launch_kry_widen(const float* e, double* z, size_t cnt, const Ctrl* ctrl, hipStream_t st);
hipError_t launch_kry_arm(const KryDev& K, Ctrl* ctrl, bool reopen, hipStream_t st);

struct EigBlocks {
    const double* p[3] = {nullptr, nullptr, nullptr};
    int nb = 0;
};
constexpr int EIG_TILE = 64;
constexpr int EIG_MAX_GROUPS = 256;
int eig_groups(int n);
size_t eig_gram_part_size(int a, int b, int groups);
hipError_t launch_eig_gram(const EigBlocks& Sa, const EigBlocks& Sb, int n, int m, const double* w, bool sym, double* part, int groups,
                           double* G, const Ctrl* ctrl, hipStream_t st);
hipError_t launch_eig_combine(const EigBlocks& S, const EigBlocks& AS, int n, int m, const double* C, double* X, double* AX, double* P,
                              double* AP, const Ctrl* ctrl, hipStream_t st);
hipError_t launch_eig_residual(const double* X, const double* AX, const double* mass, const double* lam, int n, int m, double* b0, double* u0,
                               float* b32, float* u32, double* part, int groups, double* res, const Ctrl* ctrl, hipStream_t st);

hipError_t launch_dense_gemv_add(const double* Ainv, int n, int lda, const double* b, double* u, int k, int ld,
                                 const Ctrl* ctrl, hipStream_t st, double* sym_work = nullptr);
hipError_t launch_dense_gemv_add_f32(const float* Ainv, int n, int lda, const float* b, float* u, int k, int ld,
                                     const Ctrl* ctrl, hipStream_t st, float* sym_work = nullptr);
hipError_t launch_sym_gemv_tiles(const double* Ainv, int lda, const double* b, double* part, hipStream_t st);
hipError_t launch_sym_gemv_tiles_f32(const float* Ainv, int lda, const float* b, float* part, hipStream_t st);
hipError_t launch_cvt_f64_f32(float* dst, const double* src, size_t n, hipStream_t st);
hipError_t launch_residual_to_f32(float* b32, float* u32, const double* r64, size_t n, const Ctrl* ctrl, hipStream_t st);
hipError_t launch_add_correction(double* z, const float* e, size_t n, const Ctrl* ctrl, hipStream_t st);
hipError_t launch_spd_inverse(double* M, int n, double* work, hipStream_t st);

hipError_t launch_recipe(int n_out, const int* ptr, const int* idx, const double* coef, const double* src, double* out, hipStream_t st);
hipError_t launch_sell_fill(const int* ptr, const int* col, const double* val, const int* perm, const int* iperm, const SellDev& S, size_t padded, hipStream_t st,
                            bool transposed = false);
hipError_t launch_sell_encode(const SellDev& S, size_t padded, const double* tab, int n_tab, int* out_col, int* bad, hipStream_t st);
hipError_t launch_sell_diag_slots(const SellDev& S, int* slot, int* first_missing, hipStream_t st);
hipError_t warm_device_code(hipStream_t st);
hipError_t launch_sell_fill_map(const int* ptr, const int* col, const int* perm, const int* iperm, const SellDev& S, size_t padded, bool transposed, int* map, hipStream_t st);
hipError_t launch_bit_symmetric(int n, const int* ptr, const int* col, const double* val, int* differs, hipStream_t st);
hipError_t launch_gather_vals(double* dst, const double* src, const int* map, size_t n, hipStream_t st);
hipError_t launch_dense_from_csr(double* dense, int np, int n, const double* src, const long long* pos, int nnz, hipStream_t st);
hipError_t launch_add_at(double* v, const int* where, int n, double c, hipStream_t st);

hipError_t launch_assemble(int nV, int nF, int nnz, const double* V, const int* F, int voronoi, const int* l_ptr, const int* l_idx,
                           const signed char* l_sgn, const int* m_ptr, const int* m_idx, const int* diag_of, double* Qc, double* Qm,
                           double* Md, double mass_coef, double lap_coef, double* val, double* Lval, hipStream_t st);

hipError_t launch_gather_in(double* dst, const double* src, const int* map, int n, int k, int kin, int ld_src,
                            hipStream_t st);
hipError_t launch_scatter_out(double* dst, const double* src, const int* map, int n, int k, int kin, int ld_dst,
                              hipStream_t st);
hipError_t launch_scatter_cm(double* dst, const double* src, const int* idx, int n, int k, int ld_src, int ld_dst,
                             hipStream_t st);
hipError_t launch_gather_cm(double* dst, const double* src, const int* idx, int n, int k, int ld_src, int ld_dst,
                            hipStream_t st);
hipError_t launch_csr_sub(int n_rows, const int* ptr, const int* col, const double* val, const double* x, int ldx,
                          double* y, int ld, int k, hipStream_t st);

hipError_t launch_geo_basis(const double* V, const int* F, int nF, double* W, double* Af, hipStream_t st);
hipError_t launch_geo_scatter(int n, int k, const int* src_ptr, const int* src, double* B, int ldb, hipStream_t st);
hipError_t launch_geo_divergence(int n, int k, const int* F, const double* W, const double* Af, const int* m_ptr, const int* m_idx,
                                 const double* U, int ldu, double* out, int ldo, hipStream_t st);
hipError_t launch_geo_shift(int n, int k, const int* src_ptr, const int* src, const double* phi, int ldp, double* mean, double* D, int ldd,
                            hipStream_t st);

hipError_t launch_arap_covariance(int n, const int* rowptr, const int* col, const double* w, const double* P0, const double* P, double* S, hipStream_t st);
hipError_t launch_arap_rotations(int n, const int* rowptr, const int* col, const double* w, const double* P0, const double* P, double* R, double* eterm,
                                 hipStream_t st);
hipError_t launch_arap_vertex_energy(int n, const int* rowptr, const int* col, const double* w, const double* P0, const double* P, const double* R,
                                     double* eterm, hipStream_t st);
hipError_t launch_arap_rhs(int n, const int* rowptr, const int* col, const double* w, const double* P0, const double* R, double* B, int ldb, hipStream_t st);
int arap_groups(int n);
hipError_t launch_arap_energy(const double* eterm, int n, double* part, double* E, hipStream_t st);
hipError_t launch_arap_rows(int n, const double* U, int ldu, double* P, hipStream_t st);
hipError_t launch_arap_columns(int n, const double* P, double* U, int ldu, hipStream_t st);
hipError_t launch_arap_set_handles(int nh, const int* handles, const double* hp, int ldh, double* U, int ldu, hipStream_t st);

hipError_t launch_membrane_rest(int nF, const int* F, const double* V0, double thickness, double* rest, hipStream_t st);
hipError_t launch_membrane_faces(int mode, int nF, const int* F, const double* P, const double* rest, double alpha, double beta, double floor,
                                 double value, double* W, double* G, double* H, hipStream_t st);
hipError_t launch_membrane_matrix(int nB, const int* brow, const int* bcol, const int* bptr, const int* c_ptr, const int* c_src, const double* H,
                                  int nF, double dt2, const double* mass0, double mass_scale, double* val, hipStream_t st);
hipError_t launch_membrane_pressure(int nV, int nF, const int* F, const double* P, const int* m_ptr, const int* m_idx, double pressure, double* Qn,
                                    double* mass, double* fext, hipStream_t st);
hipError_t launch_membrane_gradient(int nV, const int* m_ptr, const int* m_idx, const double* G, int nF, const double* mass0, double mass_scale,
                                    double dt, const double* qdot, const double* qdot0, const double* fext, double* g, double* b, hipStream_t st);
hipError_t launch_membrane_trial(int nV, const double* qdot, const double* dx, double step, const double* qdot0, const double* pos0,
                                 const double* fext, const double* mass0, double mass_scale, double dt, double* t_out, double* p_out, double* term,
                                 hipStream_t st);
hipError_t launch_membrane_dot3(int nV, const double* a, const double* b, double* term, hipStream_t st);

}
```

surface_multigrid_code_amd/csrc/smg_hier.hpp:

```cpp
#pragma once
#include <memory>
#include <hip/hip_runtime_api.h>

#include <atomic>
#include <cstdint>
#include <string>
#include <vector>

#include "smg_bsr3.hpp"
#include "smg_coarse.hpp"
#include "smg_device.hpp"
#include "smg_mesh.hpp"
#include "smg_order.hpp"
#include "smg_sparse.hpp"
#include "smg_tiled.hpp"
#include "smg_bgs.hpp"
#include "smg_wgs.hpp"
#include "smg_schur.hpp"

namespace smg {

inline std::atomic<long long>& devbuf_live_bytes() { static std::atomic<long long> v{0}; return v; }

template <typename T>
// ... 12 lines not shown
        hipError_t e = hipHostMalloc((void**)&p, count * sizeof(T), hipHostMallocDefault);
        if (e == hipSuccess) n = count; else p = nullptr;
        return e;
    }
};

template <typename T>
struct DevBuf {
    T* p = nullptr;
    size_t n = 0;
    DevBuf() = default;
    DevBuf(const DevBuf&) = delete;
    DevBuf& operator=(const DevBuf&) = delete;
    DevBuf(DevBuf&& o) noexcept : p(o.p), n(o.n) { o.p = nullptr; o.n = 0; }
    DevBuf& operator=(DevBuf&& o) noexcept { if (this != &o) { release(); p = o.p; n = o.n; o.p = nullptr; o.n = 0; } return *this; }
    ~DevBuf() { release(); }
    void release() { if (p) { (void)hipFree(p); devbuf_live_bytes() -= (long long)(n * sizeof(T)); } p = nullptr; n = 0; }
    hipError_t alloc(size_t count)
    {
        release();
        if (count == 0) return hipSuccess;
        hipError_t e = hipMalloc((void**)&p, count * sizeof(T));
        if (e == hipSuccess) { n = count; devbuf_live_bytes() += (long long)(count * sizeof(T)); } else p = nullptr;
        return e;
    }
    hipError_t ensure(size_t count) { return count <= n ? hipSuccess : alloc(count); }
    long long bytes() const { return (long long)(n * sizeof(T)); }
    template <class Alloc>
    hipError_t upload(const std::vector<T, Alloc>& v)
    {
        hipError_t e = alloc(v.size());
        if (e != hipSuccess || v.empty()) return e;
        return hipMemcpy(p, v.data(), v.size() * sizeof(T), hipMemcpyHostToDevice);
    }
    template <class Alloc>
    hipError_t upload_in_place(const std::vector<T, Alloc>& v, bool* moved)
    {
        if (p && v.size() == n) return v.empty() ? hipSuccess : hipMemcpy(p, v.data(), v.size() * sizeof(T), hipMemcpyHostToDevice);
        *moved = true;
        return upload(v);
    }
};

struct SellBuf {
    DevBuf<int> slice_row, slice_off, slice_w, col, order;
    DevBuf<double> val;
    SellDev view;
    std::vector<int> color_slice_ptr;
    DevBuf<int> diag_slot;
    int n_first = 0;
    int n_all = 0;
    long stored = 0, padded = 0, used = 0;
    hipError_t upload(const Sell& S);
    DevBuf<int> long_row, long_ptr, long_col;
    DevBuf<double> long_val;
    DevBuf<float> long_valf;
    hipError_t upload_long(const std::vector<int>& rows, const std::vector<int>& ptr, const std::vector<int>& col, const std::vector<double>& val);
    hipError_t encode_codes(const double* vals, size_t n_vals, hipStream_t st);
};

struct Bsr3Buf {
    DevBuf<int> slice_row, slice_off, slice_w, col, order;
    DevBuf<double> val;
    DevBuf<float> valf;
    Bsr3Dev view;
    std::vector<int> color_slice_ptr;
    long stored = 0, blocks = 0, padded = 0;
    hipError_t upload(const Bsr3Sell& S);
};

struct PlanValues {
    DevBuf<double> val, diag;
    DevBuf<int> map, mapd;
    std::vector<int> host_map, host_mapd;
    long long bytes() const { return val.bytes() + diag.bytes() + map.bytes() + mapd.bytes(); }
};

struct TiledBuf {
    DevBuf<int> hdr, ext_rows, pcol, prow;
    PlanValues v;
    TiledDev view;
    bool tried = false;
    long long bytes() const { return hdr.bytes() + ext_rows.bytes() + pcol.bytes() + prow.bytes() + v.bytes(); }
};

struct BgsBuf {
    DevBuf<int> hdr, xrow, ugrow, ulrow, eidx;
    PlanValues v;
    BgsDev view;
    std::vector<int> color_ptr;
    std::vector<int> host_rows, host_blk_ptr;
    double rim = 0.0, fill = 0.0;
    bool tried = false;
    long long bytes() const { return hdr.bytes() + xrow.bytes() + ugrow.bytes() + ulrow.bytes() + eidx.bytes() + v.bytes(); }
};

struct WgsBuf {
    DevBuf<int> hdr, grow, meta, rim;
    DevBuf<unsigned> eoff;
    PlanValues v;
    WgsDev view;
    std::vector<int> color_ptr;
    std::vector<int> host_rows, host_piece_ptr;
    double rim_ratio = 0.0, phases_mean = 0.0;
    int phases_max = 0;
    bool tried = false;
    long long bytes() const { return hdr.bytes() + grow.bytes() + meta.bytes() + rim.bytes() + eoff.bytes() + v.bytes(); }
};

struct Level {
    std::vector<double> V;
    std::vector<int> F;
    Csr P_full;
    std::shared_ptr<DecimationLog> dec_log;
    Csr A;
    std::vector<double> A_diag;
    Csr P, PT;
    Ordering ord;
    uint64_t ord_key = 0;
    Csr A_int, P_int, PT_int;
    Ordering vord;
    Csr Pv, PTv;
    Bsr3Buf bA, bAT;
    DevBuf<int> mapB, mapBT;
    SellBuf dA, dP, dPT;
    SellBuf dAT;
    bool gs_on_transpose = false;
    bool P_device_filled = false, PT_device_filled = false;
    bool device_filled = false;
    Csr vpat;
    bool A_bit_symmetric = false;
    TiledBuf tiled[4];
    WgsBuf wgs;
    BgsBuf bgs;
    std::vector<int> A_int_src;
    DevBuf<double> d_Aval;
    DevBuf<double> d_Tval;
    DevBuf<int> mapA, mapAT;
    DevBuf<int> r1_ptr, r1_idx, r2_ptr, r2_idx;
    DevBuf<double> r1_coef, r2_coef;
    int nnzT = 0;
    DevBuf<float> a32, at32, p32, pt32;
    SellDev dA32, dAT32, dP32, dPT32;
    DevBuf<float> b32, u32, r32;
    DevBuf<double> b, u, r;
    DevBuf<double> t;
    DevBuf<float> t32;
    DevBuf<double> d;
    DevBuf<float> d32;
    double lam = 0.0;
    int n = 0;
};

struct GraphKey {
    int k = 0, k_user = 0, pre = 0, post = 0, precision = 0, smoother = 0, jacobi_max_rows = 0;
    double omega = 0.0, cheby_fraction = 0.0;
    bool head_fuse = false;
    bool operator==(const GraphKey& o) const
    {
        return k == o.k && k_user == o.k_user && pre == o.pre && post == o.post && precision == o.precision && smoother == o.smoother &&
               jacobi_max_rows == o.jacobi_max_rows && omega == o.omega && cheby_fraction == o.cheby_fraction && head_fuse == o.head_fuse;
    }
    bool operator!=(const GraphKey& o) const { return !(*this == o); }
};

enum Step { STEP_ITER,
            STEP_ITER_N,
            STEP_HEAD,
            STEP_TAIL,
            STEP_SPLIT_RESID,
            STEP_SPLIT_CYCLE,
            STEP_SPEC,
            STEP_PCG,
            STEP_PCG_N,
            STEP_COUNT };

struct GraphCache {
    hipGraphExec_t exec[STEP_COUNT] = {};
    GraphKey mg_key, pcg_key;
    double* sumsq = nullptr;
    void drop(int s0 = 0, int s1 = STEP_COUNT)
    {
        for (int s = s0; s < s1; s++) if (exec[s]) { (void)hipGraphExecDestroy(exec[s]); exec[s] = nullptr; }
        if (s0 <= STEP_ITER && s1 > STEP_ITER) mg_key = GraphKey();
        if (s0 <= STEP_PCG && s1 > STEP_PCG) pcg_key = GraphKey();
    }
};

struct ProfScope { std::string name; long count = 0; double ms = 0.0; };
struct ProfRec { int scope; hipEvent_t e0, e1; };

}

struct smg_hierarchy {
    int n_levels = 0;
    std::vector<smg::Level> lv;
    int n_full = 0;
    bool has_known = false, precomputed = false;
    std::vector<int> known, unknown;
    smg::Csr LHS_unused;
    smg::Csr Auk;
    smg::DevBuf<int> d_map0;
    smg::DevBuf<int> d_perm0;
    smg::DevBuf<int> d_unknown, d_known;
    smg::DevBuf<int> d_auk_ptr, d_auk_col;
    smg::DevBuf<double> d_auk_val;
    uint64_t pre_key = 0;
    int p_version = 0;
    bool input_canonical = false;
    bool recipes_built = false, host_stale = false;
    int nnz_input = 0;
    std::vector<int> lhs_src, auk_src;
    smg::DevBuf<int> d_lhs_src, d_auk_src, d_diag_idx;
    smg::DevBuf<long long> d_dense_pos;
    smg::DevBuf<double> d_Afull;
    struct EarlyUpload { smg::DevBuf<int> ptr, col; smg::DevBuf<double> val; bool valid = false; } early0;
// ... 91 lines not shown
```

surface_multigrid_code_amd/csrc/smg_internal.hpp:

```cpp
#pragma once
#include <hip/hip_runtime_api.h>

#include <chrono>
#include <cstdio>
#include <cstdlib>
#include <exception>
#include <new>
#include <string>

#include "../../include/smg.h"
#include "smg_hier.hpp"
#include "smg_mesh.hpp"

namespace smg {

int fail(int code, const char* fmt, ...) __attribute__((format(printf, 2, 3)));

#define HIPCHK(expr)                                                                                          \
    do {                                                                                                      \
        hipError_t e__ = (expr);                                                                              \
        if (e__ != hipSuccess) return ::smg::fail(SMG_ERR_HIP, "%s failed: %s", #expr, hipGetErrorString(e__)); \
    } while (0)

template <typename Fn>
// ... 54 lines not shown
void prof_collect(smg_hierarchy* h);
struct ProfGuard {
    smg_hierarchy* h; int idx = -1;
    ProfGuard(smg_hierarchy* hh, const char* name) : h(hh)
    {
        if (!h->prof_on) return;
        ProfRec r; r.scope = prof_scope_id(h, name); r.e0 = prof_event(h); r.e1 = prof_event(h);
        (void)hipEventRecord(r.e0, h->stream);
        h->recs.push_back(r);
        idx = (int)h->recs.size() - 1;
    }
    ~ProfGuard() { if (idx >= 0) (void)hipEventRecord(h->recs[idx].e1, h->stream); }
};

const char* check_compressed(int n_major, int n_minor, const int* ptr, const int* idx);
int set_prolong(smg_hierarchy* h, int lv, Csr&& P);
Mesh wrap_mesh(const double* V, int nV, const int* F, int nF);

double double_area(const double* V, const int* F, int f);
int components(const int* F, int nF, int nV);
int level0_rows(const smg_hierarchy* h);
long long handle_bytes(const smg_hierarchy* h);
int copy_prolongations(const smg_hierarchy* src, smg_hierarchy* dst);

struct MembraneLists { std::vector<int> bptr, bcol, brow, c_ptr, c_src; };
void membrane_lists(const int* F, int nF, int nV, MembraneLists& L);

int spectral_bounds(smg_hierarchy* h);
int ensure_spectral_bounds(smg_hierarchy* h);
int refresh_host_values(smg_hierarchy* h);
int ensure_P_int(smg_hierarchy* h, int lv);
int ensure_A_int(smg_hierarchy* h, int lv);

int union_coarse_factor(smg_hierarchy* h, const double* d_vals, bool first);
int union_begin_solve(smg_hierarchy* h, int k);

enum { LV_GS = 0, LV_JACOBI = 1, LV_CHEBY = 2 };
int level_kind(const smg_hierarchy* h, int lv);
inline bool level_is_jacobi(const smg_hierarchy* h, int lv) { return level_kind(h, lv) != LV_GS; }

enum { FIRST_NONE = 0,
       FIRST_LAUNCH = 1,
       FIRST_SWEEP = 2 };

int ensure_work(smg_hierarchy* h, int k);
int ensure_fp32(smg_hierarchy* h, int k);
int enqueue_vcycle(smg_hierarchy* h, int k, const Ctrl* ctrl, int first);
int enqueue_residual_ss(smg_hierarchy* h, int k, bool fuse_decide = false, double* sumsq_out = nullptr);
int enqueue_cycle_part(smg_hierarchy* h, int k, const double* d_sumsq);
int apply_A(smg_hierarchy* h, int lv, SellMode mode, const double* x, const double* b, double* y, int k, const Ctrl* ctrl);
bool head_fusable(smg_hierarchy* h, int k);
int internal_cols(const smg_hierarchy* h, int k);
int coarse_stall_check(smg_hierarchy* h);

template <typename Fn>
static int capture_graph(smg_hierarchy* h, hipGraphExec_t* out, Fn&& body)
{
    hipGraph_t g = nullptr;
    HIPCHK(hipStreamBeginCapture(h->stream, hipStreamCaptureModeThreadLocal));
    int rc = body();
    hipError_t e = hipStreamEndCapture(h->stream, &g);
    if (rc) { if (g) (void)hipGraphDestroy(g); return rc; }
    if (e != hipSuccess) return fail(SMG_ERR_HIP, "hipStreamEndCapture: %s", hipGetErrorString(e));
    e = hipGraphInstantiate(out, g, nullptr, nullptr, 0);
    (void)hipGraphDestroy(g);
    if (e != hipSuccess) return fail(SMG_ERR_HIP, "hipGraphInstantiate: %s", hipGetErrorString(e));
    return SMG_OK;
}

int latch_solve_opts(smg_hierarchy* h, const smg_solve_opts& o);
int reset_ctrl(smg_hierarchy* h, int cap);

struct SweepPlan {
    const TiledDev* tiled = nullptr;
    const WgsBuf* wave = nullptr;
    const BgsBuf* block = nullptr;
    bool colours() const { return !tiled && !wave && !block; }
};
SweepPlan sweep_plan(const smg_hierarchy* h, int lv, int k, int sweeps, bool fp64, int first);
int prepare_sweep_plans(smg_hierarchy* h, int k, int sa, int sb);
int prepare_level_plans(smg_hierarchy* h, int lv);
int refresh_plan_values(smg_hierarchy* h);
void drop_sweep_plans(smg_hierarchy* h);

}
```

surface_multigrid_code_amd/csrc/smg_sweep_plans.cpp:

```cpp
#include <algorithm>
#include <climits>
#include <cmath>
#include <vector>

#include "smg_internal.hpp"

using namespace smg;

static bool gs_plan_level(const smg_hierarchy* h, int lv)
{
    return h->bs == 1 && lv >= 0 && lv < h->n_levels - 1 && level_kind(h, lv) == LV_GS;
}

static int wgs_mode_now(const smg_hierarchy* h)
{
    static const int env = env_int("SMG_WGS", -1);
    return env >= 0 ? (env == 0 ? 0 : env == 1 ? -1 : 1) : h->wgs_mode;
}
static bool wgs_in_range(const smg_hierarchy* h, int lv)
{
    static const int max_rows = env_int("SMG_WGS_MAX_ROWS", 600000), min_rows = env_int("SMG_WGS_MIN_ROWS", 512);
    return h->precision == 0 && gs_plan_level(h, lv) && h->lv[lv].n >= min_rows && h->lv[lv].n <= max_rows;
}
static bool wgs_forced(const smg_hierarchy* h, int lv) { return wgs_mode_now(h) == 1 && wgs_in_range(h, lv); }
// ... 82 lines not shown
    return h->host_stale && Lv.d_Aval.p ? gather_plan_values(h, Lv, V) : SMG_OK;
}

static int ensure_tiled(smg_hierarchy* h, int lv, int sweeps)
{
    Level& Lv = h->lv[lv];
    TiledBuf& B = Lv.tiled[sweeps];
    if (B.tried) return SMG_OK;
    B.tried = true;
    static const int rows_env = env_int("SMG_TILED_ROWS", 0), nt_env = env_int("SMG_TILED_NT", 0);
    const int tile_rows0 = rows_env > 0 ? rows_env : std::min(512, std::max(256, (Lv.n + 239) / 240));
    constexpr int max_ext = (64 * 1024 - TILED_LDS_STATIC) / 8;
    SweepMatrix M;
    { int rc = sweep_matrix(h, lv, &M); if (rc) return rc; }
    TiledGs P;
    int threads = 512;
    for (int tile_rows = tile_rows0, tries = 0; tries < 3 && P.empty(); tile_rows = tile_rows * 2 / 3, tries++) {
        threads = nt_env > 0 ? nt_env : 512;
        P = build_tiled_gs(*M.G, Lv.ord.color_ptr, sweeps, tile_rows, max_ext, threads);
    }
    if (P.empty()) return SMG_OK;
    HIPCHK(B.hdr.upload(P.hdr)); HIPCHK(B.ext_rows.upload(P.ext_rows)); HIPCHK(B.pcol.upload(P.pcol)); HIPCHK(B.prow.upload(P.prow));
    { int rc = set_plan_values(h, Lv, M, B.v, P.pval, P.pentry, P.pdiag, P.pdentry); if (rc) return rc; }
    HIPCHK(tiled_gs_prepare(P.max_ext));
    int wmax = 0;
    for (int t = 0; t < P.n_tiles; t++) wmax = std::max(wmax, P.hdr[(size_t)t * TILED_HDR + 2]);
    B.view.threads = threads;
    B.view.n_tiles = P.n_tiles; B.view.nc = P.nc; B.view.P = P.P; B.view.sweeps = sweeps; B.view.max_ext = P.max_ext; B.view.w_max = wmax;
    B.view.hdr = B.hdr.p; B.view.ext_rows = B.ext_rows.p; B.view.pcol = B.pcol.p; B.view.pval = B.v.val.p; B.view.prow = B.prow.p; B.view.pdiag = B.v.diag.p;
    if (env_int("SMG_DEBUG_TILED", 0))
        std::fprintf(stderr, "tiled relax(%d) level %d: %d rows, %d tiles x %d threads, %d phases, extended tile <= %d rows, %.2fx row updates, entries per row <= %d\n", sweeps, lv, Lv.n,
                     P.n_tiles, threads, P.P, P.max_ext, (double)P.updates / ((double)sweeps * Lv.n), wmax);
    return SMG_OK;
}

static int ensure_bgs(smg_hierarchy* h, int lv)
{
    Level& Lv = h->lv[lv];
    BgsBuf& B = Lv.bgs;
    if (B.tried) return SMG_OK;
    B.tried = true;
    static const int rows_env = env_int("SMG_BGS_ROWS", 64);
    SweepMatrix M;
    { int rc = sweep_matrix(h, lv, &M); if (rc) return rc; }
    const auto t_plan0 = std::chrono::steady_clock::now();
    BgsPlan P = build_bgs(*M.G, Lv.ord.color_ptr, std::min(std::max(rows_env, 8), (int)BGS_ROWS));
    const double plan_ms = 1e3 * std::chrono::duration<double>(std::chrono::steady_clock::now() - t_plan0).count();
    if (P.empty()) return SMG_OK;
    HIPCHK(B.hdr.upload(P.hdr)); HIPCHK(B.xrow.upload(P.xrow)); HIPCHK(B.ugrow.upload(P.ugrow)); HIPCHK(B.ulrow.upload(P.ulrow)); HIPCHK(B.eidx.upload(P.eidx));
    { int rc = set_plan_values(h, Lv, M, B.v, P.eval, P.eentry, P.udiag, P.dentry); if (rc) return rc; }
    B.view.n_blocks = P.n_blocks; B.view.n_colors = P.n_colors; B.view.xrows = P.xrows;
    B.view.hdr = B.hdr.p; B.view.xrow = B.xrow.p; B.view.ugrow = B.ugrow.p; B.view.ulrow = B.ulrow.p; B.view.udiag = B.v.diag.p; B.view.eidx = B.eidx.p; B.view.eval = B.v.val.p;
    B.color_ptr = P.color_ptr; B.host_rows = P.rows; B.host_blk_ptr = P.blk_ptr; B.rim = P.rim; B.fill = P.fill;
    if (env_int("SMG_DEBUG_BGS", 0))
        std::fprintf(stderr, "block Gauss-Seidel level %d: %d rows, %d blocks in %d colours, %.0f %% of the units' row slots hold a row of their own, rim %.3f rows read per row beyond the iterate, LDS image of %d rows; plan built in %.0f ms\n",
                     lv, Lv.n, P.n_blocks, P.n_colors, 100.0 * P.fill, P.rim, P.xrows, plan_ms);
    return SMG_OK;
}

static int ensure_wgs(smg_hierarchy* h, int lv)
{
    Level& Lv = h->lv[lv];
    WgsBuf& B = Lv.wgs;
    if (B.tried) return SMG_OK;
    B.tried = true;
    static const int rows_env = env_int("SMG_WGS_ROWS", WGS_ROWS), mode_env = env_int("SMG_WGS_PIECES", 1);
    SweepMatrix M;
    { int rc = sweep_matrix(h, lv, &M); if (rc) return rc; }
    const auto t_plan0 = std::chrono::steady_clock::now();
    WgsPlan P = build_wgs(*M.G, std::min(std::max(rows_env, 8), (int)WGS_ROWS), mode_env);
    const double plan_ms = 1e3 * std::chrono::duration<double>(std::chrono::steady_clock::now() - t_plan0).count();
    if (P.empty()) return SMG_OK;
    HIPCHK(B.hdr.upload(P.hdr)); HIPCHK(B.grow.upload(P.grow)); HIPCHK(B.meta.upload(P.meta)); HIPCHK(B.rim.upload(P.rim)); HIPCHK(B.eoff.upload(P.eoff));
    { int rc = set_plan_values(h, Lv, M, B.v, P.eval, P.eentry, P.diag, P.dentry); if (rc) return rc; }
    B.view.n_pieces = P.n_pieces; B.view.n_colors = P.n_colors; B.view.rim_pitch = P.rim_pitch; B.view.nb_max = P.nb_max;
    B.view.hdr = B.hdr.p; B.view.grow = B.grow.p; B.view.meta = B.meta.p; B.view.diag = B.v.diag.p; B.view.rim = B.rim.p; B.view.eoff = B.eoff.p; B.view.eval = B.v.val.p;
    B.color_ptr = P.color_ptr; B.host_rows = P.rows; B.host_piece_ptr = P.piece_ptr; B.rim_ratio = P.rim_ratio; B.phases_mean = P.phases_mean; B.phases_max = P.phases_max;
    if (env_int("SMG_DEBUG_WGS", 0))
        std::fprintf(stderr, "wave Gauss-Seidel level %d: %d rows, %d pieces in %d colours, phases per piece %.1f (max %d), rim %.2f rows read per row beyond the iterate, rim pitch %d; plan built in %.0f ms\n",
                     lv, Lv.n, P.n_pieces, P.n_colors, P.phases_mean, P.phases_max, P.rim_ratio, P.rim_pitch, plan_ms);
    return SMG_OK;
}

static int ensure_level_plans(smg_hierarchy* h, int lv, int k, int sa, int sb, bool drop)
{
    Level& Lv = h->lv[lv];
    int rc;
    for (int sw : {sa, sb}) if (tiled_wanted(h, lv, k, sw) && (rc = ensure_tiled(h, lv, sw))) return rc;
    if (bgs_wanted(h, lv, k) && !Lv.bgs.tried) { if (drop) drop_graphs(h); if ((rc = ensure_bgs(h, lv))) return rc; }
    if (wgs_wanted(h, lv, k) && !Lv.wgs.tried && !tiled_either(h, lv, k, sa, sb)) { if (drop) drop_graphs(h); if ((rc = ensure_wgs(h, lv))) return rc; }
    return SMG_OK;
}

int smg::prepare_level_plans(smg_hierarchy* h, int lv)
{
    static const int on = env_int("SMG_EARLY_PLANS", 1), max_rows = env_int("SMG_EARLY_PLANS_MAX_ROWS", 70000);
    if (!on || lv <= 0 || lv >= h->n_levels - 1 || h->precision != 0 || h->lv[lv].n > max_rows) return SMG_OK;
    return ensure_level_plans(h, lv, 1, h->pre, h->post, false);
}

int smg::prepare_sweep_plans(smg_hierarchy* h, int k, int sa, int sb)
{
    for (int lv = 0; lv < h->n_levels - 1; lv++) {
        Level& Lv = h->lv[lv];
        int rc = ensure_level_plans(h, lv, k, sa, sb, true);
        if (rc) return rc;
        if (tiled_either(h, lv, k, sa, sb) && Lv.t.n < (size_t)Lv.n * std::max(h->kcap, 1)) {
            drop_graphs(h);
            HIPCHK(Lv.t.alloc((size_t)Lv.n * std::max(h->kcap, 1)));
            HIPCHK(hipMemsetAsync(Lv.t.p, 0, Lv.t.n * sizeof(double), h->stream));
        }
    }
    return SMG_OK;
}

int smg::refresh_plan_values(smg_hierarchy* h)
{
    for (int lv = 0; lv < h->n_levels - 1; lv++) {
        Level& Lv = h->lv[lv];
        int rc;
        for (int s = 1; s <= 3; s++) if (Lv.tiled[s].view.n_tiles > 0 && (rc = gather_plan_values(h, Lv, Lv.tiled[s].v))) return rc;
        if (Lv.wgs.view.n_pieces > 0 && (rc = gather_plan_values(h, Lv, Lv.wgs.v))) return rc;
        if (Lv.bgs.view.n_blocks > 0 && (rc = gather_plan_values(h, Lv, Lv.bgs.v))) return rc;
    }
    return SMG_OK;
}
void smg::drop_sweep_plans(smg_hierarchy* h)
{
    for (auto& Lv : h->lv) { for (auto& B : Lv.tiled) B = TiledBuf(); Lv.bgs = BgsBuf(); Lv.wgs = WgsBuf(); }
}

extern "C" int smg_hierarchy_set_block_gs(smg_hierarchy* h, int min_rows)
{
    if (!h) return fail(SMG_ERR_INVALID, "smg_hierarchy_set_block_gs: null handle");
    if (h->in_solve) return fail(SMG_ERR_INVALID, "smg_hierarchy_set_block_gs called during a split-phase solve");
    if (min_rows != h->bgs_min_rows) { h->bgs_min_rows = min_rows; if (h->stream) drop_graphs(h); }
    return SMG_OK;
}
extern "C" int smg_level_get_block_gs_order(smg_hierarchy* h, int lv, int k, int* n_blocks, int* n_colors, int* color_ptr, int* blk_ptr, int* rows, double* stats)
{
    int rc = check_ready(h, "smg_level_get_block_gs_order");
    if (rc) return rc;
    if (lv < 0 || lv >= h->n_levels || k < 1) return fail(SMG_ERR_INVALID, "smg_level_get_block_gs_order: bad level / k");
    if (!bgs_wanted(h, lv, k)) return 0;
    if (!h->lv[lv].bgs.tried) { drop_graphs(h); if ((rc = ensure_bgs(h, lv))) return rc; }
    const BgsBuf* Q = bgs_plan(h, lv, k);
    if (!Q) return 0;
    if (n_blocks) *n_blocks = Q->view.n_blocks;
    if (n_colors) *n_colors = Q->view.n_colors;
    if (color_ptr) std::copy(Q->color_ptr.begin(), Q->color_ptr.end(), color_ptr);
    if (blk_ptr) std::copy(Q->host_blk_ptr.begin(), Q->host_blk_ptr.end(), blk_ptr);
    if (rows) std::copy(Q->host_rows.begin(), Q->host_rows.end(), rows);
    if (stats) { stats[0] = Q->rim; stats[1] = Q->fill; }
    return 1;
}

extern "C" int smg_hierarchy_set_wave_gs(smg_hierarchy* h, int mode)
{
    if (!h) return fail(SMG_ERR_INVALID, "smg_hierarchy_set_wave_gs: null handle");
    if (h->in_solve) return fail(SMG_ERR_INVALID, "smg_hierarchy_set_wave_gs called during a split-phase solve");
    if (mode < -1 || mode > 1) return fail(SMG_ERR_INVALID, "smg_hierarchy_set_wave_gs: mode must be -1 (automatic), 0 (never) or 1 (every Gauss-Seidel level in range)");
    if (mode != h->wgs_mode) { h->wgs_mode = mode; if (h->stream) drop_graphs(h); }
    return SMG_OK;
}
extern "C" int smg_level_get_wave_gs_order(smg_hierarchy* h, int lv, int k, int* n_pieces, int* n_colors, int* color_ptr, int* piece_ptr, int* rows, double* stats)
{
    int rc = check_ready(h, "smg_level_get_wave_gs_order");
    if (rc) return rc;
    if (lv < 0 || lv >= h->n_levels || k < 1) return fail(SMG_ERR_INVALID, "smg_level_get_wave_gs_order: bad level / k");
    if (!wgs_wanted(h, lv, k)) return 0;
    DeviceScope dsc(h->device);
    if ((rc = prepare_sweep_plans(h, k, h->pre, h->post))) return rc;
    const WgsBuf* Q = wgs_plan(h, lv, k);
    if (!Q || tiled_either(h, lv, k, h->pre, h->post)) return 0;
    if (n_pieces) *n_pieces = Q->view.n_pieces;
    if (n_colors) *n_colors = Q->view.n_colors;
    if (color_ptr) std::copy(Q->color_ptr.begin(), Q->color_ptr.end(), color_ptr);
    if (piece_ptr) std::copy(Q->host_piece_ptr.begin(), Q->host_piece_ptr.end(), piece_ptr);
    if (rows) std::copy(Q->host_rows.begin(), Q->host_rows.end(), rows);
    if (stats) { stats[0] = Q->rim_ratio; stats[1] = Q->phases_mean; stats[2] = (double)Q->phases_max; }
    return 1;
}


static int check_level(smg_hierarchy* h, int lv, bool args_ok, const char* who, const Csr** G)
{
    if (!h || lv < 0 || lv >= h->n_levels - 1 || !args_ok) return fail(SMG_ERR_INVALID, "%s: bad arguments", who);
    int rc = ensure_A_int(h, lv);
    if (rc) return rc;
    const Level& Lv = h->lv[lv];
    if (Lv.A_int.nr != Lv.n || Lv.n == 0 || h->bs != 1) return fail(SMG_ERR_INVALID, "%s: the host half of smg_precompute has not run (scalar hierarchies only)", who);
    *G = &Lv.A_int;
    return SMG_OK;
}
static std::vector<double> check_vector(int n, bool rhs)
{
    std::vector<double> v((size_t)n);
    for (int i = 0; i < n; i++) v[(size_t)i] = rhs ? std::cos(0.11 * i) - 0.5 * std::sin(2.1 * i) : std::sin(0.37 * i) + 0.25 * std::cos(1.3 * i);
    return v;
}
static double max_diff(const std::vector<double>& y, const std::vector<double>& ref)
{
    double d = 0.0;
    for (size_t i = 0; i < y.size(); i++) d = std::max(d, std::fabs(y[i] - ref[i]));
    return d;
}
static int check_partition(const Csr& G, const char* plan, const char* part, const char* parts, int n_parts, int n_colors, const std::vector<int>& color_ptr,
                           const std::vector<int>& part_ptr, const std::vector<int>& rows, int max_rows)
{
    const int n = G.nr;
    std::vector<int> part_of((size_t)n, -1), col_of_part((size_t)n_parts, -1);
    for (int c = 0; c < n_colors; c++) for (int q = color_ptr[(size_t)c]; q < color_ptr[(size_t)c + 1]; q++) col_of_part[(size_t)q] = c;
// ... 118 lines not shown
```

Measured before the change: 3439 V-cycles/s.

## Fuse residual into last GS colour sweep and skip first-colour prolongation

The last colour launch of the final pre-smoothing Gauss-Seidel sweep now also writes the residual for its rows, computed from the just-updated value. The separate residual kernel then runs only over the head slices, since tail-colour rows need the diagonal to be their last stored entry, which is checked on the device. Prolongation-add skips the first-colour slices when post-smoothing will overwrite those rows anyway. This removes reads of A and vectors in the residual and prolongation passes, at the cost of plan-building complexity and extra kernel variants.

After: 3467 V-cycles/s, median of 6. Within noise of the previous version (+0.8%).

```diff
diff --git a/include/smg.h b/include/smg.h
--- a/include/smg.h
+++ b/include/smg.h
@@ -5,7 +5,7 @@
 extern "C" {
 #endif
 
-#define SMG_VERSION 508
+#define SMG_VERSION 509
 
 enum {
     SMG_OK = 0,
@@ -224,6 +224,7 @@
 enum { SMG_F32_RESIDUAL_TO_F32 = 0, SMG_F32_ADD_CORRECTION = 1 };
 int smg_debug_convert_f32(smg_hierarchy *h, int op, int k, int done, const double *in64, const float *in32, double *out64, float *out_b32,
                           float *out_u32, int *inputs_changed);
+int smg_debug_cycle_done(smg_hierarchy *h, int lv, int k, int pre, int post, int *vectors_written);
 enum { SMG_GEO_BASIS = 0, SMG_GEO_SCATTER = 1, SMG_GEO_DIVERGENCE = 2, SMG_GEO_SHIFT = 3 };
 int smg_debug_geodesics(int op, int n, int nF, int k, const int *F, const int *m_ptr, const int *m_idx, const int *src_ptr, const int *src,
                         const double *in, double *W, double *Af, double *out, int ld_out, int *guard_bad);
diff --git a/surface_multigrid_code_amd/_lib.py b/surface_multigrid_code_amd/_lib.py
--- a/surface_multigrid_code_amd/_lib.py
+++ b/surface_multigrid_code_amd/_lib.py
@@ -77,6 +77,7 @@
         "smg_debug_krylov": (i, [i, i, i, dp, dp, dp, dp, fp, dp, ip, d, i, dp, ip, ip, ip]),
         "smg_debug_cycle_f32": (i, [vp, i, i, i, i, i, i, fp, fp, fp, ip]),
         "smg_debug_convert_f32": (i, [vp, i, i, i, dp, fp, dp, fp, fp, ip]),
+        "smg_debug_cycle_done": (i, [vp, i, i, i, i, ip]),
         "smg_debug_geodesics": (i, [i, i, i, i, ip, ip, ip, ip, ip, dp, dp, dp, dp, i, ip]),
         "smg_geodesics_create": (i, [vp, dp, i, ip, i, d, i, C.POINTER(vp)]),
         "smg_geodesics_destroy": (None, [vp]),
diff --git a/surface_multigrid_code_amd/csrc/smg_cycle.cpp b/surface_multigrid_code_amd/csrc/smg_cycle.cpp
--- a/surface_multigrid_code_amd/csrc/smg_cycle.cpp
+++ b/surface_multigrid_code_amd/csrc/smg_cycle.cpp
@@ -278,7 +278,8 @@
 }
 
 template <typename T>
-static int enqueue_gs(smg_hierarchy* h, int lv, const SweepPlan& sp, const T* b, T* u, int k, int iters, const Ctrl* ctrl, int first = FIRST_NONE, T* t = nullptr)
+static int enqueue_gs(smg_hierarchy* h, int lv, const SweepPlan& sp, const T* b, T* u, int k, int iters, const Ctrl* ctrl, int first = FIRST_NONE, T* t = nullptr,
+                      T* r_tail = nullptr)
 {
     Level& Lv = h->lv[lv];
     ProfGuard pg(h, "MG: relaxation");
@@ -297,7 +298,11 @@
     const std::vector<int>& cs = colour_slices(h, Lv);
     for (int it = first == FIRST_SWEEP ? 1 : 0; it < iters; it++)
         for (size_t c = (it == 0 && first == FIRST_LAUNCH) ? 1 : 0; c + 1 < cs.size(); c++) {
-            if (it == 1 && first == FIRST_SWEEP) HIPCHK(Prec<T>::sell(SELL_GS_OOP, Prec<T>::G(Lv), cs[c], cs[c + 1], t, b, u, k, ctrl, h->stream));
+            if (r_tail && it == iters - 1 && c + 2 == cs.size()) {
+                const bool oop = it == 1 && first == FIRST_SWEEP;
+                HIPCHK(Prec<T>::sell(oop ? SELL_GS_OOP_TAIL : SELL_GS_TAIL, Prec<T>::G(Lv), cs[c], cs[c + 1], oop ? t : u, b, u, k, ctrl, h->stream, r_tail));
+            }
+            else if (it == 1 && first == FIRST_SWEEP) HIPCHK(Prec<T>::sell(SELL_GS_OOP, Prec<T>::G(Lv), cs[c], cs[c + 1], t, b, u, k, ctrl, h->stream));
             else HIPCHK(Prec<T>::opA(h, Lv, true, SELL_GS, cs[c], cs[c + 1], u, b, u, k, ctrl));
         }
     return SMG_OK;
@@ -362,6 +367,7 @@
     int cur = 0;
     const bool fp64 = std::is_same<T, double>::value;
     const SweepPlan sp_pre = sweep_plan(h, lv, k, pre, fp64, first), sp_post = sweep_plan(h, lv, k, post, fp64, FIRST_NONE);
+    const SellTail* tail = (fp64 && kind == LV_GS && sp_pre.colours() && h->bs == 1 && pre >= 1 && k < 8 && h->union_m == 0 && !h->prof_on) ? tail_plan(h, lv) : nullptr;
     int rc;
     if (kind == LV_JACOBI) {
         if (first_done) cur = 1;
@@ -370,11 +376,16 @@
         if (first_done) cur = 1;
         rc = enqueue_cheby<T>(h, lv, Prec<T>::b(Lv), buf, &cur, k, pre, ctrl, first_done);
     } else if (sp_pre.tiled) rc = enqueue_gs_tiled<T>(h, *sp_pre.tiled, Prec<T>::b(Lv), buf, &cur, k, ctrl);
-    else rc = enqueue_gs<T>(h, lv, sp_pre, Prec<T>::b(Lv), buf[0], k, pre, ctrl, first, buf[1]);
+    else rc = enqueue_gs<T>(h, lv, sp_pre, Prec<T>::b(Lv), buf[0], k, pre, ctrl, first, buf[1], tail ? Prec<T>::r(Lv) : nullptr);
     if (rc) return rc;
     {
         ProfGuard pg(h, "MG: residual");
-        HIPCHK(Prec<T>::opA(h, Lv, false, SELL_RESID, 0, -1, buf[cur], Prec<T>::b(Lv), Prec<T>::r(Lv), k, ctrl));
+        if (tail) {
+            SellDev head = Prec<T>::A(Lv);
+            head.n_slices = tail->n_head; head.order = tail->order.p;
+            HIPCHK(Prec<T>::sell(SELL_RESID, head, 0, head.n_slices, buf[cur], Prec<T>::b(Lv), Prec<T>::r(Lv), k, ctrl, h->stream));
+        }
+        else HIPCHK(Prec<T>::opA(h, Lv, false, SELL_RESID, 0, -1, buf[cur], Prec<T>::b(Lv), Prec<T>::r(Lv), k, ctrl));
     }
     const SellBuf& Gc = Lc.gs_on_transpose ? Lc.dAT : Lc.dA;
     const int kind_c = level_kind(h, lv + 1);
@@ -407,7 +418,14 @@
         const int flips = sp_post.tiled ? 1 : kind == LV_CHEBY ? (post > 0 ? post + 1 : 0) : post;
         if ((jac || sp_post.tiled) && ((cur + flips) & 1)) dst = 1 - cur;
         if (!jac && !sp_post.tiled && cur == 1) dst = 0;
-        HIPCHK(Prec<T>::sell(SELL_ADD, Prec<T>::P(Lc), 0, Prec<T>::P(Lc).n_slices, Prec<T>::u(Lc), buf[cur], buf[dst], kt, ctrl, h->stream));
+        const SellTail* skip = (fp64 && kind == LV_GS && post >= 1 && sp_post.colours() && h->bs == 1 && dst == 0 && cur == 0) ? prolong_skip_plan(h, lv) : nullptr;
+        if (skip) {
+            SellDev part = Prec<T>::P(Lc);
+            if (skip->p_order.p) { part.n_slices = skip->p_n; part.order = skip->p_order.p; }
+            const int s0 = skip->p_order.p ? 0 : skip->p_begin;
+            HIPCHK(Prec<T>::sell(SELL_ADD, part, s0, s0 + skip->p_n, Prec<T>::u(Lc), buf[cur], buf[dst], kt, ctrl, h->stream));
+        }
+        else HIPCHK(Prec<T>::sell(SELL_ADD, Prec<T>::P(Lc), 0, Prec<T>::P(Lc).n_slices, Prec<T>::u(Lc), buf[cur], buf[dst], kt, ctrl, h->stream));
         cur = dst;
     }
     if (kind == LV_CHEBY) return enqueue_cheby<T>(h, lv, Prec<T>::b(Lv), buf, &cur, k, post, ctrl);
@@ -900,6 +918,41 @@
     });
 }
 
+extern "C" int smg_debug_cycle_done(smg_hierarchy* h, int lv, int k, int pre, int post, int* vectors_written)
+{
+    return guarded("smg_debug_cycle_done", [&]() -> int {
+        if (!h) return fail(SMG_ERR_INVALID, "smg_debug_cycle_done: null handle");
+        if (!vectors_written || pre < 0 || post < 0) return fail(SMG_ERR_INVALID, "smg_debug_cycle_done: missing output or negative sweep count");
+        int rc = piece_prolog(h, lv, k, "smg_debug_cycle_done", false);
+        if (rc) return rc;
+        DeviceScope dsc(h->device);
+        if ((rc = prepare_sweep_plans(h, k, pre, post))) return rc;
+        HookCtrlReset reset_on_exit{h};
+        if ((rc = hook_ctrl(h, 1))) return rc;
+        constexpr int pattern = 0x3F;
+        std::vector<DevBuf<double>*> bufs;
+        for (Level& Lv : h->lv)
+            for (DevBuf<double>* b : {&Lv.b, &Lv.u, &Lv.r, &Lv.t, &Lv.d}) if (b->n) bufs.push_back(b);
+        for (DevBuf<double>* b : bufs) HIPCHK(hipMemsetAsync(b->p, pattern, b->n * sizeof(double), h->stream));
+        rc = enqueue_vcycle_t<double>(h, lv, k, pre, post, h->d_ctrl.p);
+        if (!rc && lv == 0 && pre >= 2 && h->n_levels >= 2 && h->bs == 1 && !h->lv[0].gs_on_transpose && level_kind(h, 0) == LV_GS &&
+            h->lv[0].t.n >= (size_t)h->lv[0].n * k && sweep_plan(h, 0, k, pre, true, FIRST_NONE).colours())
+            rc = enqueue_vcycle_t<double>(h, 0, k, pre, post, h->d_ctrl.p, FIRST_SWEEP);
+        int written = 0;
+        std::vector<unsigned char> now;
+        for (DevBuf<double>* b : bufs) {
+            now.resize(b->n * sizeof(double));
+            HIPCHK(hipMemcpyAsync(now.data(), b->p, now.size(), hipMemcpyDeviceToHost, h->stream));
+            HIPCHK(hipStreamSynchronize(h->stream));
+            for (unsigned char c : now) if (c != pattern) { written++; break; }
+            HIPCHK(hipMemsetAsync(b->p, 0, b->n * sizeof(double), h->stream));
+        }
+        HIPCHK(hipStreamSynchronize(h->stream));
+        *vectors_written = written;
+        return rc;
+    });
+}
+
 extern "C" int smg_debug_convert_f32(smg_hierarchy* h, int op, int k, int done, const double* in64, const float* in32, double* out64, float* out_b32,
                                      float* out_u32, int* inputs_changed)
 {
diff --git a/surface_multigrid_code_amd/csrc/smg_device.hip b/surface_multigrid_code_amd/csrc/smg_device.hip
--- a/surface_multigrid_code_amd/csrc/smg_device.hip
+++ b/surface_multigrid_code_amd/csrc/smg_device.hip
@@ -39,6 +39,7 @@
     const int wave = threadIdx.x >> 6;
     constexpr int wpb = WPB;
     constexpr bool GS = sell_is_gs(MODE), OOP = sell_is_oop(MODE), JAC = sell_is_jacobi(MODE), CHEB = sell_is_cheby(MODE), HEAD = sell_is_head(MODE);
+    constexpr bool TAIL = sell_is_tail(MODE);
     int bid;
     if (GS && n_blocks < 0) { if (blockIdx.x & 7) return; bid = blockIdx.x >> 3; }
     else bid = xcd_remap(blockIdx.x, n_blocks);
@@ -63,6 +64,7 @@
             size_t keep = (size_t)x ^ (size_t)A.slice_row ^ (size_t)A.slice_w ^ (size_t)b ^ (size_t)y ^ (size_t)done ^ (size_t)ld;
             if (MODE == SELL_AX) keep ^= (size_t)z.u ^ (size_t)z.gs_val ^ (size_t)z.diag_slot ^ (size_t)z.n_first ^ (size_t)z.jacobi ^ (size_t)z.d;
             if (CHEB) keep ^= (size_t)z.d;
+            if (TAIL) keep ^= (size_t)z.u;
             asm("" : "+s"(keep));
             if (keep == 0x5a5a5a5a5a5a5a5bull) return;
         }
@@ -75,6 +77,7 @@
         T acc[KB];
         T accr[KB];
         T diag = (T)1;
+        bool hasd = false;
         T xi[KB];
         T dold[KB];
         T bv[KB];
@@ -104,7 +107,7 @@
                 if constexpr (MODE == SELL_GS_HEAD) {
                     gather_kb<KB, T>(x + (size_t)c[t] * ld, c[t] >= 0, xo[t]);
                     gather_kb<KB, T>((const T*)y + (size_t)c[t] * ld, use && c[t] < split, xv[t]);
-                } else if constexpr (MODE == SELL_GS_OOP) {
+                } else if constexpr (MODE == SELL_GS_OOP || MODE == SELL_GS_OOP_TAIL) {
                     gather_kb<KB, T>((c[t] < split ? (const T*)y : x) + (size_t)c[t] * ld, use, xv[t]);
                 } else {
                     gather_kb<KB, T>(x + (size_t)c[t] * ld, use, xv[t]);
@@ -119,6 +122,7 @@
                     }
                     if (GS && c[t] == rowb) {
                         diag = v[t];
+                        if (TAIL) hasd = true;
                     } else if ((JAC || CHEB) && c[t] == rowb) {
                         diag = v[t];
 #pragma unroll
@@ -155,6 +159,11 @@
                 }
                 else if (MODE == SELL_RESID) y[o + q] = bv[q] - acc[q];
                 else if (MODE == SELL_ADD) y[o + q] = bv[q] + acc[q];
+                else if (TAIL) {
+                    const T yv = (bv[q] - acc[q]) / diag;
+                    y[o + q] = yv;
+                    z.u[o + q] = hasd ? bv[q] - (acc[q] + diag * yv) : bv[q] - acc[q];
+                }
                 else if (GS) y[o + q] = (bv[q] - acc[q]) / diag;
                 else if (JAC) { const T t = (bv[q] - acc[q]) / diag; y[o + q] = xi[q] + z.omega * (t - xi[q]); }
                 else if (CHEB) {
@@ -605,7 +614,9 @@
     if (ns <= 0) return hipSuccess;
     int c0 = 0;
     size_t poff = 0;
-    {
+    if constexpr (sell_is_tail(MODE)) {
+        if (k >= 8 || !zero_rows || first) return hipErrorInvalidValue;
+    } else {
         while (k - c0 >= 8) {
             int kw = 64;
             while (kw > k - c0) kw >>= 1;
@@ -697,6 +708,12 @@
             else return hipErrorInvalidValue;
         case SELL_GS_OOP:
             if constexpr (std::is_same<T, double>::value) return launch_sell_mode<SELL_GS_OOP, T>(A, s_begin, s_end, x, b, y, k, ctrl, partials, n_blocks, st, zero_rows, first, omega);
+            else return hipErrorInvalidValue;
+        case SELL_GS_TAIL:
+            if constexpr (std::is_same<T, double>::value) return launch_sell_mode<SELL_GS_TAIL, T>(A, s_begin, s_end, x, b, y, k, ctrl, partials, n_blocks, st, zero_rows, first, omega);
+            else return hipErrorInvalidValue;
+        case SELL_GS_OOP_TAIL:
+            if constexpr (std::is_same<T, double>::value) return launch_sell_mode<SELL_GS_OOP_TAIL, T>(A, s_begin, s_end, x, b, y, k, ctrl, partials, n_blocks, st, zero_rows, first, omega);
             else return hipErrorInvalidValue;
         case SELL_GS_HEAD:
             if constexpr (std::is_same<T, double>::value) return launch_sell_mode<SELL_GS_HEAD, T>(A, s_begin, s_end, x, b, y, k, ctrl, partials, n_blocks, st, zero_rows, first, omega);
@@ -1808,6 +1825,26 @@
     return hipGetLastError();
 }
 
+__global__ __launch_bounds__(256) void k_sell_tail_check(const int* __restrict__ slice_row, const int* __restrict__ slice_off, const int* __restrict__ slice_w, int stride,
+                                                         int s_begin, int s_end, const int* __restrict__ s_col, int* bad)
+{
+    const int lane = threadIdx.x & 63, s = s_begin + (int)blockIdx.x * 4 + (int)(threadIdx.x >> 6);
+    if (s >= s_end) return;
+    const int row0 = slice_row[s], nrow = slice_row[s + 1] - row0;
+    if (lane >= nrow) return;
+    const int r = row0 + lane, w = slice_w[s];
+    const size_t base = (size_t)(stride ? s * stride : slice_off[s]) * 64 + lane;
+    int last = -1;
+    for (int j = 0; j < w; j++) { const int c = s_col[base + (size_t)j * 64]; if (c >= 0) last = c; }
+    if (last != r) atomicOr(bad, 1);
+}
+hipError_t launch_sell_tail_check(const SellDev& S, int s_begin, int s_end, int* bad, hipStream_t st)
+{
+    if (s_end <= s_begin) return hipSuccess;
+    hipLaunchKernelGGL(k_sell_tail_check, dim3((s_end - s_begin + 3) / 4), dim3(256), 0, st, S.slice_row, S.slice_off, S.slice_w, S.stride, s_begin, s_end, S.col, bad);
+    return hipGetLastError();
+}
+
 __global__ void k_nothing() {}
 hipError_t warm_device_code(hipStream_t st)
 {
diff --git a/surface_multigrid_code_amd/csrc/smg_device.hpp b/surface_multigrid_code_amd/csrc/smg_device.hpp
--- a/surface_multigrid_code_amd/csrc/smg_device.hpp
+++ b/surface_multigrid_code_amd/csrc/smg_device.hpp
@@ -55,9 +55,12 @@
     SELL_GS_HEAD = 9,
     SELL_JACOBI_HEAD = 10,
     SELL_CHEBY_HEAD = 11,
-};
-constexpr bool sell_is_gs(int m) { return m == SELL_GS || m == SELL_GS_OOP || m == SELL_GS_HEAD; }
-constexpr bool sell_is_oop(int m) { return m == SELL_GS_OOP || m == SELL_GS_HEAD; }
+    SELL_GS_TAIL = 12,
+    SELL_GS_OOP_TAIL = 13,
+};
+constexpr bool sell_is_tail(int m) { return m == SELL_GS_TAIL || m == SELL_GS_OOP_TAIL; }
+constexpr bool sell_is_gs(int m) { return m == SELL_GS || m == SELL_GS_OOP || m == SELL_GS_HEAD || sell_is_tail(m); }
+constexpr bool sell_is_oop(int m) { return m == SELL_GS_OOP || m == SELL_GS_HEAD || m == SELL_GS_OOP_TAIL; }
 constexpr bool sell_is_jacobi(int m) { return m == SELL_JACOBI || m == SELL_JACOBI_HEAD; }
 constexpr bool sell_is_cheby(int m) { return m == SELL_CHEBY || m == SELL_CHEBY_HEAD; }
 constexpr bool sell_is_head(int m) { return m == SELL_GS_HEAD || m == SELL_JACOBI_HEAD || m == SELL_CHEBY_HEAD; }
@@ -248,6 +251,7 @@
                             bool transposed = false);
 hipError_t launch_sell_encode(const SellDev& S, size_t padded, const double* tab, int n_tab, int* out_col, int* bad, hipStream_t st);
 hipError_t launch_sell_diag_slots(const SellDev& S, int* slot, int* first_missing, hipStream_t st);
+hipError_t launch_sell_tail_check(const SellDev& S, int s_begin, int s_end, int* bad, hipStream_t st);
 hipError_t warm_device_code(hipStream_t st);
 hipError_t launch_sell_fill_map(const int* ptr, const int* col, const int* perm, const int* iperm, const SellDev& S, size_t padded, bool transposed, int* map, hipStream_t st);
 hipError_t launch_bit_symmetric(int n, const int* ptr, const int* col, const double* val, int* differs, hipStream_t st);
diff --git a/surface_multigrid_code_amd/csrc/smg_hier.hpp b/surface_multigrid_code_amd/csrc/smg_hier.hpp
--- a/surface_multigrid_code_amd/csrc/smg_hier.hpp
+++ b/surface_multigrid_code_amd/csrc/smg_hier.hpp
@@ -118,6 +118,17 @@
     TiledDev view;
     bool tried = false;
     long long bytes() const { return hdr.bytes() + ext_rows.bytes() + pcol.bytes() + prow.bytes() + v.bytes(); }
+};
+
+struct SellTail {
+    bool tried = false, ok = false;
+    const int* col = nullptr;
+    int n_head = 0;
+    DevBuf<int> order;
+    bool p_ok = false;
+    const int* p_col = nullptr;
+    int p_begin = 0, p_n = 0;
+    DevBuf<int> p_order;
 };
 
 struct BgsBuf {
@@ -168,6 +179,7 @@
     bool A_bit_symmetric = false;
     TiledBuf tiled[4];
     WgsBuf wgs;
+    SellTail tail;
     BgsBuf bgs;
     std::vector<int> A_int_src;
     DevBuf<double> d_Aval;
diff --git a/surface_multigrid_code_amd/csrc/smg_internal.hpp b/surface_multigrid_code_amd/csrc/smg_internal.hpp
--- a/surface_multigrid_code_amd/csrc/smg_internal.hpp
+++ b/surface_multigrid_code_amd/csrc/smg_internal.hpp
@@ -160,5 +160,7 @@
 int prepare_level_plans(smg_hierarchy* h, int lv);
 int refresh_plan_values(smg_hierarchy* h);
 void drop_sweep_plans(smg_hierarchy* h);
+const SellTail* tail_plan(const smg_hierarchy* h, int lv);
+const SellTail* prolong_skip_plan(const smg_hierarchy* h, int lv);
 
 }
diff --git a/surface_multigrid_code_amd/csrc/smg_sweep_plans.cpp b/surface_multigrid_code_amd/csrc/smg_sweep_plans.cpp
--- a/surface_multigrid_code_amd/csrc/smg_sweep_plans.cpp
+++ b/surface_multigrid_code_amd/csrc/smg_sweep_plans.cpp
@@ -188,6 +188,77 @@
     return SMG_OK;
 }
 
+static int fuse_tail_mode() { static const int v = env_int("SMG_FUSE_TAIL", 1); return v; }
+static bool fuse_tail() { return fuse_tail_mode() != 0; }
+static bool fuse_tail_resid() { return fuse_tail_mode() == 1 || fuse_tail_mode() == 2; }
+static bool fuse_tail_prolong() { return fuse_tail_mode() == 1 || fuse_tail_mode() == 3; }
+const SellTail* smg::tail_plan(const smg_hierarchy* h, int lv)
+{
+    if (!fuse_tail_resid() || h->bs != 1 || lv < 0 || lv >= h->n_levels - 1) return nullptr;
+    const Level& Lv = h->lv[lv];
+    const SellTail& T = Lv.tail;
+    return T.ok && !Lv.gs_on_transpose && T.col == Lv.dA.view.col ? &T : nullptr;
+}
+const SellTail* smg::prolong_skip_plan(const smg_hierarchy* h, int lv)
+{
+    if (!fuse_tail_prolong() || h->bs != 1 || lv < 0 || lv >= h->n_levels - 1) return nullptr;
+    const SellTail& T = h->lv[lv].tail;
+    return T.p_ok && T.p_col == h->lv[lv + 1].dP.view.col ? &T : nullptr;
+}
+static int filtered_order(smg_hierarchy* h, const int* order, int n, int lo, int hi, DevBuf<int>& out, bool* ok)
+{
+    *ok = true;
+    if (!order) return SMG_OK;
+    std::vector<int> all((size_t)n), keep;
+    HIPCHK(hipMemcpyAsync(all.data(), order, all.size() * sizeof(int), hipMemcpyDeviceToHost, h->stream));
+    HIPCHK(hipStreamSynchronize(h->stream));
+    keep.reserve((size_t)(hi - lo));
+    for (int s : all) if (s >= lo && s < hi) keep.push_back(s);
+    *ok = (int)keep.size() == hi - lo;
+    if (*ok) HIPCHK(out.upload(keep));
+    return SMG_OK;
+}
+static int ensure_tail(smg_hierarchy* h, int lv)
+{
+    Level& Lv = h->lv[lv];
+    SellTail& T = Lv.tail;
+    if (T.tried) return SMG_OK;
+    T.tried = true; T.ok = false; T.p_ok = false;
+    if (!fuse_tail() || h->bs != 1) return SMG_OK;
+    const SellDev& V = Lv.dA.view;
+    const std::vector<int>& cs = Lv.dA.color_slice_ptr;
+    const int n_head = cs.size() >= 3 ? cs[cs.size() - 2] : 0;
+    if (!Lv.gs_on_transpose && n_head > 0 && n_head < V.n_slices && V.col && V.val && !V.codes && V.long_n == 0 && V.n_rows == V.n_cols && cs.back() == V.n_slices) {
+        DevBuf<int> d_bad;
+        int bad = 0;
+        HIPCHK(d_bad.alloc(1));
+        HIPCHK(hipMemsetAsync(d_bad.p, 0, sizeof(int), h->stream));
+        HIPCHK(launch_sell_tail_check(V, n_head, V.n_slices, d_bad.p, h->stream));
+        HIPCHK(hipMemcpyAsync(&bad, d_bad.p, sizeof(int), hipMemcpyDeviceToHost, h->stream));
+        HIPCHK(hipStreamSynchronize(h->stream));
+        bool ok = false;
+        if (!bad) { int rc = filtered_order(h, V.order, V.n_slices, 0, n_head, T.order, &ok); if (rc) return rc; }
+        if (ok) { T.col = V.col; T.n_head = n_head; T.ok = true; }
+    }
+    const SellBuf& P = h->lv[lv + 1].dP;
+    const std::vector<int>& cp = Lv.ord.color_ptr;
+    if (cp.size() >= 3 && P.view.col && P.view.C == 64 && P.view.n_rows == Lv.n && P.view.long_n == 0 && P.view.n_slices > 0) {
+        int begin = -1;
+        if (P.color_slice_ptr.size() == cp.size()) begin = P.color_slice_ptr[1];
+        else if (P.color_slice_ptr.size() == 2) begin = cp[1] / 64;
+        if (begin > 0 && begin < P.view.n_slices) {
+            bool ok = false;
+            int rc = filtered_order(h, P.view.order, P.view.n_slices, begin, P.view.n_slices, T.p_order, &ok);
+            if (rc) return rc;
+            if (ok) { T.p_col = P.view.col; T.p_begin = begin; T.p_n = P.view.n_slices - begin; T.p_ok = true; }
+        }
+    }
+    if (env_int("SMG_DEBUG_TAIL", 0))
+        std::fprintf(stderr, "tail fusion level %d: %d rows, residual out of the last colour launch %s (residual launch: %d of %d slices), prolongation %s (from slice %d of %d)\n", lv,
+                     Lv.n, T.ok ? "on" : "off", T.ok ? T.n_head : V.n_slices, V.n_slices, T.p_ok ? "without the first colour" : "whole", T.p_ok ? T.p_begin : 0, P.view.n_slices);
+    return SMG_OK;
+}
+
 static int ensure_level_plans(smg_hierarchy* h, int lv, int k, int sa, int sb, bool drop)
 {
     Level& Lv = h->lv[lv];
@@ -211,6 +282,7 @@
         Level& Lv = h->lv[lv];
         int rc = ensure_level_plans(h, lv, k, sa, sb, true);
         if (rc) return rc;
+        if ((rc = ensure_tail(h, lv))) return rc;
         if (tiled_either(h, lv, k, sa, sb) && Lv.t.n < (size_t)Lv.n * std::max(h->kcap, 1)) {
             drop_graphs(h);
             HIPCHK(Lv.t.alloc((size_t)Lv.n * std::max(h->kcap, 1)));
@@ -233,7 +305,7 @@
 }
 void smg::drop_sweep_plans(smg_hierarchy* h)
 {
-    for (auto& Lv : h->lv) { for (auto& B : Lv.tiled) B = TiledBuf(); Lv.bgs = BgsBuf(); Lv.wgs = WgsBuf(); }
+    for (auto& Lv : h->lv) { for (auto& B : Lv.tiled) B = TiledBuf(); Lv.bgs = BgsBuf(); Lv.wgs = WgsBuf(); Lv.tail = SellTail(); }
 }
 
 extern "C" int smg_hierarchy_set_block_gs(smg_hierarchy* h, int min_rows)
```
